# mojing1999/jmcodec

Hardware: AMD Instinct MI355X
Metric: decoded frames/sec @1080p H.264 + bit-exact YUV (higher is better)
Workload: dtype u8

## Files before the change

### jmcodec_amd/csrc/deblock_lds.hip

```cpp
#include <hip/hip_runtime.h>
#include <cstdlib>
#include <algorithm>
#include "jobs.h"
#include "kernels.h"
#include "kernel_common.h"
#include "deblock_device.h"

namespace jmamd {

__global__ __launch_bounds__(256) void k_deblock_prep(const PicParams *pics) {
    const PicParams &pp = pics[blockIdx.y];
    if (!(pp.stages & (PS_DEBLOCK_LDS | PS_CHAIN))) return;
    DbRec *out = (DbRec *)pp.dbrec;
    const int per_xcd = ((int)gridDim.x + 7) >> 3;
    const int blk = ((int)blockIdx.x & 7) * per_xcd + ((int)blockIdx.x >> 3);
    __shared__ __align__(16) uint8_t stage[8][96];
    int sub = threadIdx.x >> 5, t = threadIdx.x & 31;
    int mb = blk * 8 + sub;
    int n_mbs = pp.mb_w * pp.mb_h;
    if (mb >= n_mbs) return;
    int mbx = mb % pp.mb_w, mby = mb / pp.mb_w;
    const MbW q = load_mbw(&pp.mbs[mb]);
    const SliceRec sl = pp.slices[mbw_slice(q)];
    bool has_left = mbx > 0, has_top = mby > 0;
    MbW pl = q, pt = q;
    if (has_left) { pl = load_mbw(&pp.mbs[mb - 1]); if (sl.disable == 2 && mbw_slice(pl) != mbw_slice(q)) has_left = false; }
    if (has_top) { pt = load_mbw(&pp.mbs[mb - pp.mb_w]); if (sl.disable == 2 && mbw_slice(pt) != mbw_slice(q)) has_top = false; }
    int dir = t >> 4, e = (t >> 2) & 3, k = t & 3;
    int rq = dir == 0 ? k * 4 + e : e * 4 + k;
    int bs;
    if (sl.disable == 1) bs = 0;
    else if (e == 0) {
        bool have = dir == 0 ? has_left : has_top;
        const MbW pn = select_mbw(dir == 0, pl, pt);
        bs = have ? boundary_strength(pp, pn, dir == 0 ? k * 4 + 3 : 12 + k, q, rq, true, dir == 1) : 0;
    } else bs = boundary_strength(pp, q, dir == 0 ? rq - 1 : rq - 4, q, rq, false, dir == 1);
    if ((e & 1) && (mbw_modes(q) & MBM_T8X8)) bs = 0;
    int cls = e ? 1 : (dir ? 2 : 0);
    int qp_p = cls == 0 ? mbw_qp(pl) : (cls == 2 ? mbw_qp(pt) : mbw_qp(q)), qp_q = mbw_qp(q);
    DbRec *o = (DbRec *)stage[sub];
    {
        int qpav = (qp_p + qp_q + 1) >> 1;
        int ia = clip3(0, 51, qpav + sl.alpha_off), ib = clip3(0, 51, qpav + sl.beta_off);
        int tc0 = (bs >= 1 && bs <= 3) ? kTc0[ia][bs - 1] : 0;
        o->y_bs[t] = (uint8_t)(bs | (tc0 << 3));
        if (k == 0 && (e == 0 || (e == 1 && dir == 0))) { o->y_ab[cls][0] = kAlpha[ia]; o->y_ab[cls][1] = kBeta[ib]; }
    }
    if (!(e & 1)) {
#pragma unroll
        for (int plane = 0; plane < 2; plane++) {
            int off = plane ? pp.cr_qp_off : pp.cb_qp_off;
            int qpav = (chroma_qp(qp_p, off) + chroma_qp(qp_q, off) + 1) >> 1;
            int ia = clip3(0, 51, qpav + sl.alpha_off), ib = clip3(0, 51, qpav + sl.beta_off);
            int tc0 = (bs >= 1 && bs <= 3) ? kTc0[ia][bs - 1] : 0;
            o->c_bs[plane][dir * 8 + (e >> 1) * 4 + k] = (uint8_t)(bs | (tc0 << 3));
            if (k == 0 && (e == 0 || (e == 2 && dir == 0))) { o->c_ab[plane][cls][0] = kAlpha[ia]; o->c_ab[plane][cls][1] = kBeta[ib]; }
        }
    }
    if (t < 6) ((uint4 *)&out[mb])[t] = ((const uint4 *)stage[sub])[t];
}

template <int DEPTH>
__global__ __launch_bounds__(kBandRows * 16) void k_deblock_band(const PicParams *pics, int *ctl, int pub, int *err) {
    __shared__ __align__(16) uint8_t smem[kDeblockSmemBytes];
    const PicParams &pp = pics[blockIdx.y];
    if (!(pp.stages & PS_DEBLOCK_LDS)) return;
    deblock_band_body<DEPTH, false>(pp, blockIdx.x >> 1, blockIdx.x & 1, ctl + (size_t)blockIdx.y * kChainStride + kChainRing, pub, smem, nullptr,
        err + blockIdx.y);
}

bool deblock_lds_supported(int mb_w, int mb_h) { return mb_w > 0 && mb_h <= kBandRows * kDeblockMaxBands; }

constexpr int kDeblockDepth = 2, kDeblockPub = 2;
int deblock_depth() { return kDeblockDepth; }
int deblock_row_lag() { return kRowLag; }
int deblock_pub() { return kDeblockPub; }

void launch_deblock_prep(const PicParams *d_pics, int n, int max_mbs, hipStream_t st) {
    hipLaunchKernelGGL(k_deblock_prep, dim3(((max_mbs + 7) / 8 + 7) & ~7, n), dim3(256), 0, st, d_pics);
}
void launch_deblock_lds(const PicParams *d_pics, int n, int max_mb_h, int *ctl, int *err, bool debug_stall, hipStream_t st) {
    const int depth = deblock_depth(), pub = debug_stall ? -1 : deblock_pub();
    const int bands = (max_mb_h + kBandRows - 1) / kBandRows;
    dim3 grid(2 * bands, n), block(kBandRows * 16);
    if (depth <= 2) hipLaunchKernelGGL((k_deblock_band<2>), grid, block, 0, st, d_pics, ctl, pub, err);
    else if (depth == 3) hipLaunchKernelGGL((k_deblock_band<3>), grid, block, 0, st, d_pics, ctl, pub, err);
    else hipLaunchKernelGGL((k_deblock_band<4>), grid, block, 0, st, d_pics, ctl, pub, err);
}

}
```

### jmcodec_amd/csrc/decoder.cpp

```cpp
#include "decoder.h"
#include "numa.h"
#include <pthread.h>
#include <time.h>
#include "engine.h"
#include "host_copy.h"
#include "kernels.h"
#include <hip/hip_runtime_api.h>
#include <algorithm>
#include <cstdio>
#include <cstdlib>
#include <cstring>
#include <thread>

namespace jmamd {

#define HIP_OK(expr) ((expr) == hipSuccess)

namespace {
int thread_budget() {
    const char *e = getenv("JM_AMD_DEC_THREADS");
    int n = e ? atoi(e) : (int)std::thread::hardware_concurrency();
    if (!e) {
        if (FILE *f = fopen("/sys/fs/cgroup/cpu.max", "r")) {
            long long q = 0, per = 0; char qs[32] = {0};
            if (fscanf(f, "%31s %lld", qs, &per) == 2 && strcmp(qs, "max") != 0 && per > 0) { q = atoll(qs); int lim = (int)((q * 5 / 4 + per - 1) / per);
                if (lim < 4) lim = 4; if (n > lim) n = lim; }
            fclose(f);
        }
    }
    return std::max(1, std::min(n, 64));
}
struct Pool {
    std::mutex m; std::condition_variable cv;
    std::deque<std::pair<Decoder *, PicTask *>> q;
    std::vector<std::thread> threads;
    int n = 0, node = -1; bool bound = false;
    Pool(int node_, int n_) : n(n_), node(node_) {
        bound = (int)numa_cpus_of_node(node).size() >= std::max(2, (n * 4 / 5 + 1) / 2);
        for (int i = 0; i < n; i++) threads.emplace_back([this] { pthread_setname_np(pthread_self(),
            "jm-parse"); if (bound) numa_bind_this_thread(node); run(); });
        for (auto &t : threads) t.detach();
    }
    void run() {
        ParseScratch scratch;
        for (;;) {
            std::pair<Decoder *, PicTask *> job;
            { std::unique_lock<std::mutex> lk(m); cv.wait(lk, [&] { return !q.empty(); }); job = q.front(); q.pop_front(); }
            try { job.first->parse_task(job.second, scratch); }
            catch (const std::exception &e) { job.first->parse_exception(job.second, e.what()); }
            catch (...) { job.first->parse_exception(job.second, "unknown exception"); }
        }
    }
};
std::mutex g_pools_m;
std::vector<Pool *> g_pools;
Pool &pool_of_node(int node) {
    std::lock_guard<std::mutex> lk(g_pools_m);
    for (Pool *p : g_pools) if (p->node == node) return *p;
    int n = thread_budget();
    if (node >= 0 && !getenv("JM_AMD_DEC_DEVICE")) {
        cpu_set_t allowed; CPU_ZERO(&allowed);
        const int total = sched_getaffinity(0, sizeof allowed, &allowed) == 0 ? CPU_COUNT(&allowed) : 0;
        const int mine = (int)numa_cpus_of_node(node).size();
        if (total > 0 && mine > 0 && mine < total) n = std::max(2, (n * mine + total - 1) / total);
    }
    g_pools.push_back(new Pool(node, n));
    return *g_pools.back();
}
std::atomic<int> g_handle_counter{0};
std::atomic<int> g_handle_index{0};
}

void pool_submit(Decoder *d, PicTask *t) { Pool &p = pool_of_node(d->numa_node()); { std::lock_guard<std::mutex> lk(p.m); p.q.emplace_back(d, t); }
    p.cv.notify_one(); }
int pool_threads(int node) { return pool_of_node(node).n; }

static long long now_ns() { return std::chrono::duration_cast<std::chrono::nanoseconds>(std::chrono::steady_clock::now().time_since_epoch()).count(); }

Decoder::Decoder() { memset(info_, 0, sizeof info_); trace_on_ = getenv("JM_AMD_DEC_TRACE") != nullptr; eng_state_ = new EngineDecoderState(); }

Decoder::~Decoder() {
    { std::unique_lock<std::mutex> lk(mtx_); cv_.wait(lk, [&] { return outstanding_ == 0 && parse_pending_ == 0; }); }
    { std::lock_guard<std::mutex> lk(submit_mtx_); }
    if (copier_) { copier_->free_signal(out_sig_); out_sig_ = 0; }
    gpu_close();
    delete eng_state_;
    if (trace_on_ && !trace_.empty()) {
        char name[256]; snprintf(name, sizeof name, "%s.%p.csv", getenv("JM_AMD_DEC_TRACE"), (void *)this);
        if (FILE *f = fopen(name, "w")) {
            fprintf(f, "seq,is_i,dispatch,parsed,submit0,submit1\n");
            for (auto &r : trace_)
                fprintf(f, "%llu,%d,%lld,%lld,%lld,%lld\n", (unsigned long long)r.seq, r.is_i, r.t_dispatch, r.t_parsed, r.t_submit0, r.t_submit1);
            fclose(f);
        }
    }
}

void Decoder::fail(const std::string &msg) {
    std::lock_guard<std::mutex> lk(error_m_);
    if (!failed_) { error_ = msg; fprintf(stderr, "jm_amd_dec: %s\n", msg.c_str()); }
    failed_ = true;
}
const char *Decoder::last_error() {
    std::lock_guard<std::mutex> lk(error_m_);
    error_out_ = error_;
    return error_out_.c_str();
}

void Decoder::note_error(const std::string &msg) {
    std::lock_guard<std::mutex> lk(error_m_);
    if (!failed_) error_ = msg;
}

int Decoder::set_option(const char *key, long long v) {
    std::string k(key);
    if (k == "parse_only") parse_only_ = v != 0;
    else if (k == "digest") { want_digest_ = v != 0; if (want_digest_) sync_mode_ = true; }
    else if (k == "display_delay") display_delay_ = (int)std::max(0ll, std::min(v, (long long)n_jobs_ - 4));
    else if (k == "job_slots") { if (inited_) return -1; n_jobs_ = (int)std::max(8ll, std::min(v, (long long)kMaxJobSlots)); n_jobs_set_ = true; }
    else if (k == "fast_parse") fast_parse_ = v != 0;
    else if (k == "job_digest") { want_job_digest_ = v != 0; if (want_job_digest_) sync_mode_ = true; }
    else if (k == "sync") sync_mode_ = v != 0;
    else if (k == "device_output") device_output_ = v != 0;
    else if (k == "device") device_ = (int)v;
    else if (k == "crop_x" || k == "crop_y" || k == "crop_w" || k == "crop_h" || k == "target_width" || k == "target_height") {
        if (inited_ || v < 0 || v > 32768 || (v & 1)) return -1;
        static const char *const keys[6] = {"crop_x", "crop_y", "crop_w", "crop_h", "target_width", "target_height"};
        for (int i = 0; i < 6; i++) if (k == keys[i]) geo_[i] = (int)v;
    }
    else if (k == "rect_x" || k == "rect_y" || k == "rect_w" || k == "rect_h") {
        if (inited_ || v < 0 || v > 32768 || (v & 1)) return -1;
        rect_opt_[k[5] == 'x' ? 0 : k[5] == 'y' ? 1 : k[5] == 'w' ? 2 : 3] = (int)v;
    }
    else if (k == "fit") { if (inited_ || v < 0 || v > 2) return -1; fit_ = (int)v; }
    else if (k == "fit_sar") { if (inited_ || v < 0 || v > 1) return -1; fit_sar_ = (int)v; }
    else if (k == "fill") { if (inited_ || v < -1 || v > 0xFFFFFF) return -1; fill_ = v; }
    else if (k == "deinterlace" || k == "deinterlace_when" || k == "deinterlace_field" || k == "deinterlace_threshold") {
        const long long hi = k == "deinterlace" || k == "deinterlace_field" ? 2 : (k == "deinterlace_when" ? 1 : 255);
        if (inited_ || v < 0 || v > hi) return -1;
        (k == "deinterlace" ? deint_mode_ : k == "deinterlace_when" ? deint_when_ : k == "deinterlace_field" ? deint_field_ : deint_thr_) = (int)v;
    }
    else if (k == "deinterlace_rate") {
        if (inited_ || v < 0 || v > 1) return -1;
        deint_rate_ = (int)v;
    }
    else if (k == "verify_hash") {
        if (inited_ || v < 0 || v > 2) return -1;
        verify_hash_ = (int)v;
    }
    else if (k == "verify_md5") {
        if (inited_ || v < 0 || v > 1) return -1;
        verify_md5_ = (int)v;
    }
    else if (k == "rgb_chroma") {
        if (inited_ || v < 0 || v > 1) return -1;
        rgb_chroma_ = (int)v;
    }
    else if (k == "chroma_loc") {
        if (inited_ || v < -1 || v > 5) return -1;
        chroma_loc_opt_ = (int)v;
    }
    else if (k == "profile") { profile_ = v != 0; if (engine_) engine_->set_profile(profile_); }
    else if (k.rfind("chain_", 0) == 0 || k == "debug_stall" || k == "debug_no_bi" || k == "early_intra_ahead") {
        if (!engine_ || !engine_->set_knob(k, v)) return -1;
    }
    else if (k == "wait_idle") {
        dispatch_pending();
        { std::unique_lock<std::mutex> lk(mtx_); cv_.wait(lk, [&] { return outstanding_ == 0; }); }
    }
    else return -1;
    return 0;
}
long long Decoder::get_stat(const char *key) const {
    std::string k(key);
    if (k == "inferred_frames") return stat_inferred_frames_.load();
    if (k == "redundant_slices") return stat_redundant_slices_.load();
    if (k == "field_pictures") return stat_field_pics_.load();
    if (k == "lone_fields") return stat_lone_fields_.load();
    if (k == "frames") return num_frames_;
    if (k == "out_width") return out_w_;
    if (k == "out_height") return out_h_;
    if (k == "rect_x") return place_[0];
    if (k == "rect_y") return place_[1];
    if (k == "rect_w") return place_[2];
    if (k == "rect_h") return place_[3];
    if (k == "placed_frames") return stat_placed_;
    if (k == "sar_num") return sar_[0];
    if (k == "sar_den") return sar_[1];
    if (k == "scaled_frames") return stat_scaled_;
    if (k == "rgb_frames") return stat_rgb_;
    if (k == "deint_frames") return stat_deint_;
    if (k == "field_rate_pairs") return stat_pairs_;
    if (k == "interlaced_sequence") return codec_ == 0 && seq_active_ && !seq_.frame_mbs_only ? 1 : 0;
    if (k == "out_frame_bytes") { std::lock_guard<std::mutex> lk(const_cast<std::mutex &>(mtx_));
        return (long long)(cur_out_ ? cur_out_->fbytes : !ready_.empty() ? ready_.front()->fbytes : frame_bytes_); }
    if (k == "out_slot_bytes") { std::lock_guard<std::mutex> lk(const_cast<std::mutex &>(mtx_)); long long n = 0;
        for (const OutSlot *o : all_out_) n += (o->host ? (long long)o->bytes : 0) + (o->dev ? (long long)o->bytes : 0); return n; }
    if (k == "vui_full_range") return vui_[0];
    if (k == "vui_primaries") return vui_[1];
    if (k == "vui_transfer") return vui_[2];
    if (k == "vui_matrix") return vui_[3];
    if (k == "color_matrix") return color_matrix_;
    if (k == "color_range") return color_range_;
    if (k == "vui_chroma_loc") return vui_chroma_loc_[0];
    if (k == "vui_chroma_loc_bottom") return vui_chroma_loc_[1];
    if (k == "chroma_loc") return chroma_loc_;
    if (k == "rgb_chroma") return rgb_chroma_;
    if (k == "rgb_chroma_frames") return stat_rgb_chroma_;
    if (k == "pictures") return stat_pictures_;
    if (k == "hash_pictures") return stat_hash_pics_;
    if (k == "hash_checked") return stat_hash_checked_;
    if (k == "hash_mismatch") return stat_hash_mismatch_;
    if (k == "hash_unchecked") return stat_hash_unchecked_;
    if (k == "hash_md5") return stat_hash_md5_;
    if (k == "hash_first_bad_poc") return stat_hash_bad_poc_;
    if (k.rfind("hash_last_crc:", 0) == 0 || k.rfind("hash_last_checksum:", 0) == 0) {
        const bool crc = k[10] == 'c' && k[11] == 'r'; const int c = atoi(k.c_str() + (crc ? 14 : 19));
        return c >= 0 && c < 3 ? (long long)hash_last_[(crc ? 0 : 3) + c].load() : -1; }
    if (k.rfind("hash_last_md5:", 0) == 0) {
        const size_t c2 = k.find(':', 14); if (c2 == std::string::npos) return -1;
        const int c = atoi(k.c_str() + 14), w = atoi(k.c_str() + c2 + 1);
        return c >= 0 && c < 3 && w >= 0 && w < 4 ? (long long)hash_last_md5_[4 * c + w].load() : -1;
    }
    if (k.rfind("hash_sei_", 0) == 0) {
        const size_t colon = k.find(':'); if (colon == std::string::npos) return -1;
        const size_t i = (size_t)atoll(k.c_str() + colon + 1); if (i >= hash_seen_.size()) return -1;
        if (k.compare(0, colon, "hash_sei_md5") == 0) {
            const size_t c2 = k.find(':', colon + 1), c3 = c2 == std::string::npos ? c2 : k.find(':', c2 + 1);
            if (c3 == std::string::npos) return -1;
            const int c = atoi(k.c_str() + c2 + 1), w = atoi(k.c_str() + c3 + 1);
            if (c < 0 || c > 2 || w < 0 || w > 3) return -1;
            const uint8_t *d = hash_seen_[i].h.md5[c] + 4 * w;
            return (long long)((uint32_t)d[0] << 24 | (uint32_t)d[1] << 16 | (uint32_t)d[2] << 8 | d[3]);
        }
        if (k.compare(0, colon, "hash_sei_poc") == 0) return hash_seen_[i].poc;
        if (k.compare(0, colon, "hash_sei_type") == 0) return hash_seen_[i].h.type;
        const size_t c2 = k.find(':', colon + 1);
        if (k.compare(0, colon, "hash_sei_value") == 0 && c2 != std::string::npos) { const int c = atoi(k.c_str() + c2 + 1);
            return c >= 0 && c < 3 ? (long long)hash_seen_[i].h.v[c] : -1; }
        return -1;
    }
    if (k == "job_bytes") return stat_job_bytes_;
    if (k == "job_regrown") return stat_job_regrown_;
    if (k == "job_slot_bytes") { long long n = 0; for (auto &j : jobs_) n += (long long)j.cap; return n; }
    if (k == "errors") return stat_errors_;
    if (k == "failed") return failed_ ? 1 : 0;
    if (k == "jpeg_pictures") return stat_jpeg_pics_;
    if (k == "jpeg_sampling") return codec_ == 2 && seq_active_ ? j_sampling_ : 0;
    if (k == "jpeg_restart_intervals") return stat_jpeg_ri_;
    if (k == "copy_engines") return copier_ ? (long long)copier_->engine_mask() : 0;
    if (k == "direct_frames") return stat_direct_;
    if (k == "direct_ns") return stat_direct_ns_;
    if (k == "device_wait_errors") return stat_wait_errors_;
    if (k == "intra_mbs") return stat_intra_mbs_;
    if (k == "coef_int16") return stat_coef_;
    if (k == "syntax_digest") return codec_ == 1 ? (long long)hdigest_.h : (long long)digest_.h;
    if (k == "job_digest") return (long long)job_digest_;
    if (k == "digest_mbs") return codec_ == 1 ? (long long)hdigest_.n_cu : (long long)digest_.mbs;
    if (k == "i_pictures") return stat_i_;
    if (k == "p_pictures") return stat_p_;
    if (k == "b_pictures") return stat_b_;
    if (k == "fps_num") return codec_ == 1 ? (long long)hsps_.time_scale : (long long)seq_.time_scale;
    if (k == "fps_den") return codec_ == 1 ? (long long)hsps_.num_units_in_tick : 2ll * seq_.num_units_in_tick;
    if (k == "out_fps_num") { const bool chosen = deint_when_ == 1 || (codec_ == 0 && seq_active_ && !seq_.frame_mbs_only);
        return (field_rate() && chosen ? 2 : 1) * get_stat("fps_num"); }
    if (k == "out_fps_den") return get_stat("fps_den");
    if (k == "frames_done_unfetched") return (long long)frames_done_unfetched();
    if (k == "frames_waiting") { std::lock_guard<std::mutex> lk(const_cast<std::mutex &>(mtx_)); return (long long)ready_.size(); }
    if (k == "pictures_in_flight") { std::lock_guard<std::mutex> lk(const_cast<std::mutex &>(mtx_)); return (long long)outstanding_; }
    if (k == "coded_width") return mb_w_ * 16;
    if (k == "coded_height") return mb_h_ * 16;
    if (k == "pitch") return pitch_;
    if (k == "device") return device_;
    if (k == "threads") return pool_threads(numa_node_);
    if (k == "numa_node") return numa_node_;
    if (k == "elapsed_us") return (long long)(elapsed_ms_ * 1000.0);
    if (k == "parse_ns_i") return stat_parse_ns_i_;
    if (k == "submit_ns") return stat_submit_ns_;
    if (k == "wait_slot_ns") return stat_wait_slot_ns_;
    if (k == "parse_ns_p") return stat_parse_ns_p_;
    if (k.rfind("k_", 0) == 0 || k.rfind("eng_", 0) == 0) {
        static const char *kn[kKernelClasses] = {"inter", "intra", "deblock", "packout", "chain", "rgb_pack", "deint", "jpeg", "pichash", "md5", "rgb_pack444"};
        if (!engine_) return 0;
        EngineStats es = engine_->stats();
        for (int i = 0; i < kKernelClasses; i++) {
            if (k == std::string("k_") + kn[i] + "_ns") return (long long)es.ns[i];
            if (k == std::string("k_") + kn[i] + "_n") return es.launches[i];
            if (k == std::string("k_") + kn[i] + "_pics") return es.pics[i];
            if (k == std::string("k_") + kn[i] + "_alg_bytes") return es.alg_bytes[i];
        }
        if (k == "eng_batches") return es.batches;
        if (k == "eng_forms") return es.forms;
        if (k == "eng_form_decoders") return es.form_decoders;
        if (k == "eng_form_pending") return es.form_pending;
        if (k == "eng_batch_pics") return es.batch_pics;
        if (k == "eng_chain_batches") return es.chain_batches;
        if (k == "eng_chain_pics") return es.chain_pics;
        if (k == "eng_chain_i_batches") return es.chain_i_batches;
        if (k == "eng_wait_errors") return es.wait_errors;
        if (k == "eng_chain_recoveries") return es.chain_recoveries;
        if (k == "eng_gpu_shared") return engine_->gpu_shared() ? 1 : 0;
        if (k == "eng_launch_ns") return es.launch_ns;
        if (k == "eng_wait_gap_launches") return es.wait_gap_launches;
        if (k == "eng_wait_gap_max_us") return es.wait_gap_max_ticks / 100;
        if (k == "eng_quad_windows") return es.quad_windows;
        if (k == "eng_private_windows") return es.private_windows;
        if (k == "eng_rej_other_lane") return es.rej_other_lane;
        if (k == "eng_rej_cross_lane") return es.rej_cross_lane;
        if (k == "eng_rej_tables") return es.rej_tables;
        if (k == "eng_early_intra") return es.early_intra;
        if (k == "eng_blocked_ns") return es.blocked_ns;
        if (k == "eng_blocked_n") return es.blocked_n;
        for (int i = 0; i < 4; i++) {
            const std::string l = std::to_string(i);
            if (k == "eng_lane" + l + "_busy_ns") return (long long)es.lane_busy_ns[i];
            if (k == "eng_lane" + l + "_gap_ns") return (long long)es.lane_gap_ns[i];
            if (k == "eng_lane" + l + "_upwait_ns") return (long long)es.lane_upwait_ns[i];
            if (k == "eng_lane" + l + "_prewait_ns") return (long long)es.lane_prewait_ns[i];
            if (k == "eng_lane" + l + "_dry") return es.lane_dry[i];
            if (k == "eng_lane" + l + "_batches") return es.lane_batches[i];
            if (k == "eng_lane" + l + "_pics") return es.lane_pics[i];
        }
        if (k == "eng_complete_ns") return es.complete_ns;
        return -1;
    }
    if (k.rfind("display_field:", 0) == 0) { size_t i = (size_t)atoll(k.c_str() + 14);
        return i < display_fields_.size() ? display_fields_[i] : (i < display_pocs_.size() ? 0 : -1); }
    if (k.rfind("display_picture:", 0) == 0) { size_t i = (size_t)atoll(k.c_str() + 16);
        if (field_rate()) return i < display_pics_.size() ? (long long)display_pics_[i] : -1;
        return i < display_pocs_.size() ? (long long)i : -1; }
    if (k.rfind("display_poc:", 0) == 0) { size_t i = (size_t)atoll(k.c_str() + 12); return i < display_pocs_.size() ? display_pocs_[i] : -1; }
    return -1;
}

int Decoder::init(int codec_type, int out_fmt, const uint8_t *extra, int len) {
    codec_ = codec_type; out_fmt_ = out_fmt ? 1 : 0;
    if (codec_type != 0 && codec_type != 1 && codec_type != 2) { fail("only codec_type 0 (H.264), 1 (HEVC) and 2 (MJPEG) are implemented"); return -1; }
    if (rgb_chroma_ && !rgb_) { fail("option rgb_chroma needs RGB output: set an RGB spec (jm_amddec_set_rgb) before init"); return -1; }
    if (getenv("JM_AMD_DEC_SYNC")) sync_mode_ = true;
    if (const char *js = getenv("JM_AMD_DEC_JOB_SLOTS")) { n_jobs_ = std::max(8, std::min(atoi(js), kMaxJobSlots)); n_jobs_set_ = true; }
    if (const char *dd = getenv("JM_AMD_DEC_DISPLAY_DELAY")) display_delay_ = std::max(0, std::min(atoi(dd), n_jobs_ - 4));
    if (getenv("JM_AMD_DEC_PARSE_ONLY")) parse_only_ = true;
    out_via_copy_engine_ = !getenv("JM_AMD_DEC_OUT_DIRECT");
    if (getenv("JM_AMD_DEC_DEVICE_OUTPUT")) device_output_ = true;
    cavlc_init_tables();
    if (parse_only_) numa_node_ = numa_node_of_device(device_ < 0 ? 0 : device_, false);
    if (!parse_only_ && !gpu_open()) return -1;
    {
        int fa = 2, fb = 5;
        const char *e = getenv("JM_AMD_DEC_OUT_FETCH");
        out_route_ = 3;
        if (getenv("JM_AMD_DEC_OUT_PINNED") || !out_via_copy_engine_) out_route_ = 2;
        else if (e && !strcmp(e, "auto")) out_route_ = 0;
        else if (e && strcmp(e, "direct")) { if (sscanf(e, "%d/%d", &fa, &fb) != 2 || fb <= 0) { fa = 2; fb = 5; }
            out_route_ = (handle_index_ % fb) < fa ? 1 : 2; }
        if (out_route_ == 3 && !parse_only_) {
            copier_ = HostCopier::get(device_);
            if (copier_) out_sig_ = copier_->new_signal();
            if (!copier_ || !out_sig_) { copier_ = nullptr; out_route_ = (handle_index_ % 5) < 2 ? 1 : 2; }
        }
        out_fetch_ = out_route_ == 1 || out_route_ == 3;
        if (const char *l = getenv("JM_AMD_DEC_FETCH_LIMIT")) fetch_limit_ = atoi(l);
    }
    if (engine_) engine_->set_profile(profile_);
    inited_ = true;
    if (extra && len > 0 && codec_ == 1 && len >= 23 && extra[0] == 1) {
        avcc_len_size_ = (extra[21] & 3) + 1;
        int o = 23;
        for (int a = 0, n_arrays = extra[22]; a < n_arrays && o + 3 <= len; a++) {
            int n = (extra[o + 1] << 8) | extra[o + 2]; o += 3;
            for (int i = 0; i < n && o + 2 <= len; i++) {
                int l = (extra[o] << 8) | extra[o + 1]; o += 2;
                if (l <= 0 || o + l > len) { o = len; break; }
                handle_nal(extra + o, (size_t)l); o += l;
            }
        }
    } else if (extra && len > 0) {
        if (len >= 7 && extra[0] == 1) {
            avcc_len_size_ = (extra[4] & 3) + 1;
            int o = 5, n_sps = extra[o++] & 31;
            for (int pass = 0; pass < 2; pass++) {
                int n = pass == 0 ? n_sps : (o < len ? extra[o++] : 0);
                for (int i = 0; i < n && o + 2 <= len; i++) {
                    int l = (extra[o] << 8) | extra[o + 1]; o += 2;
                    if (l <= 0 || o + l > len) { o = len; break; }
                    handle_nal(extra + o, (size_t)l); o += l;
                }
            }
        } else { feed(extra, (size_t)len); static const uint8_t sc[4] = {0, 0, 0, 1}; feed(sc, 4); in_.clear(); scan_ = 0; have_start_ = false; }
    }
    return 0;
}

bool Decoder::gpu_open() {
    int n = 0;
    if (!HIP_OK(hipGetDeviceCount(&n)) || n <= 0) { fail("no HIP device available (the HIP backend is mandatory; there is no CPU fallback)"); return false; }
    if (device_ < 0) {
        const char *e = getenv("JM_AMD_DEC_DEVICE");
        device_ = e ? atoi(e) : (g_handle_counter++ % n);
    }
    const int named_device = device_;
    if (device_ >= n) device_ %= n;
    mem_trace("handle: before hipSetDevice");
    if (!HIP_OK(hipSetDevice(device_))) { fail("hipSetDevice failed"); return false; }
    mem_trace("handle: hipSetDevice");
    handle_index_ = g_handle_index++;
    numa_node_ = numa_node_of_device(getenv("JM_AMD_DEC_FAKE_NUMA") ? named_device : device_, true);
    engine_ = Engine::get(device_);
    if (!engine_) { fail("could not start the device engine (stream / buffer creation failed)"); return false; }
    gpu_open_ = true;
    mem_trace("handle: engine ready");
    return true;
}

void Decoder::free_job_buffers() {
    for (auto &j : jobs_) {
        if (j.big >= 0) { j.host = j.own_host; j.dev = j.own_dev; j.big = -1; }
        if (gpu_open_ && !parse_only_) { if (j.host) hipHostFree(j.host); if (j.dev) hipFree(j.dev); if (j.dbrec) hipFree(j.dbrec);
            if (j.resid) hipFree(j.resid); if (j.uploaded) hipEventDestroy(j.uploaded); }
        else free(j.host);
        j = JobSlot();
    }
    for (auto &b : big_) {
        if (gpu_open_ && !parse_only_) { if (b.host) hipHostFree(b.host); if (b.dev) hipFree(b.dev); } else free(b.host);
        b = BigJobBuf();
    }
}

void Decoder::free_surfaces() {
    if (surf_block_) hipFree(surf_block_);
    surf_block_ = nullptr;
    for (auto &p : surf_) p = nullptr;
}

void Decoder::gpu_free_sequence() {
    if (!gpu_open_) return;
    hipSetDevice(device_);
    free_surfaces();
    if (resid_) { hipFree(resid_); resid_ = nullptr; }
    for (auto &w : hevc_work_) if (w) { hipFree(w); w = nullptr; }
    if (hevc_bs_) { hipFree(hevc_bs_); hevc_bs_ = nullptr; }
    if (scale_dev_) { hipFree(scale_dev_); scale_dev_ = nullptr; }
    if (chroma_dev_) { hipFree(chroma_dev_); chroma_dev_ = nullptr; }
    free_job_buffers();
    free_out_slots(true);
}
void Decoder::free_out_slots(bool all) {
    std::lock_guard<std::mutex> lk(mtx_);
    std::vector<OutSlot *> keep;
    for (OutSlot *o : all_out_) {
        bool pending = !all && (o == cur_out_ || std::find(ready_.begin(), ready_.end(), o) != ready_.end());
        if (pending) { keep.push_back(o); continue; }
        if (o->host) hipHostFree(o->host);
        if (o->dev) hipFree(o->dev);
        delete o;
    }
    all_out_ = keep; free_out_.clear();
    if (all) { ready_.clear(); done_unfetched_ = 0; cur_out_ = nullptr; }
}
void Decoder::gpu_close() {
    if (!gpu_open_) { for (OutSlot *o : all_out_) delete o; all_out_.clear(); free_job_buffers(); return; }
    gpu_free_sequence();
    gpu_open_ = false;
}

bool upload_scale_tables(int w, int h, int tw, int th, uint8_t **dev, ScaleAxis ax[4]) {
    const int S[4] = {w, h, w / 2, h / 2}, D[4] = {tw, th, tw / 2, th / 2};
    std::vector<int32_t> first[4]; std::vector<int16_t> wt[4];
    size_t off[4][2], total = 0;
    for (int a = 0; a < 4; a++) {
        const int T = build_scale_taps(S[a], D[a], first[a], wt[a]);
        if (T < 0 || T > kScaleMaxTaps) return false;
        ax[a].taps = T; ax[a].src_len = S[a];
        off[a][0] = total; total += (first[a].size() * sizeof(int32_t) + 255) & ~(size_t)255;
        off[a][1] = total; total += (wt[a].size() * sizeof(int16_t) + 255) & ~(size_t)255;
    }
    std::vector<uint8_t> host(total, 0);
    for (int a = 0; a < 4; a++) { memcpy(host.data() + off[a][0], first[a].data(), first[a].size() * sizeof(int32_t));
        memcpy(host.data() + off[a][1], wt[a].data(), wt[a].size() * sizeof(int16_t)); }
    *dev = nullptr;
    if (!HIP_OK(hipMalloc((void **)dev, total))) { *dev = nullptr; return false; }
    if (!HIP_OK(hipMemcpy(*dev, host.data(), total, hipMemcpyHostToDevice))) { hipFree(*dev); *dev = nullptr; return false; }
    for (int a = 0; a < 4; a++) { ax[a].first = (const int32_t *)(*dev + off[a][0]); ax[a].w = (const int16_t *)(*dev + off[a][1]); }
    return true;
}

bool upload_chroma_tables(int w, int h, int tw, int th, int loc, uint8_t **dev, ScaleAxis cax[2]) {
    if (loc < 0 || loc > 5) return false;
    const int S[2] = {w / 2, h / 2}, D[2] = {tw, th}, q[2] = {chr::siting_qx(loc), chr::siting_qy(loc)};
    std::vector<int32_t> first[2]; std::vector<int16_t> wt[2];
    size_t off[2][2], total = 0;
    for (int a = 0; a < 2; a++) {
        const int T = build_chroma_taps(S[a], D[a], q[a], first[a], wt[a]);
        if (T < 0 || T > chr::kChromaMaxTaps) return false;
        cax[a].taps = T; cax[a].src_len = S[a];
        off[a][0] = total; total += (first[a].size() * sizeof(int32_t) + 255) & ~(size_t)255;
        off[a][1] = total; total += (wt[a].size() * sizeof(int16_t) + 255) & ~(size_t)255;
    }
    std::vector<uint8_t> host(total, 0);
    for (int a = 0; a < 2; a++) { memcpy(host.data() + off[a][0], first[a].data(), first[a].size() * sizeof(int32_t));
        memcpy(host.data() + off[a][1], wt[a].data(), wt[a].size() * sizeof(int16_t)); }
    *dev = nullptr;
    if (!HIP_OK(hipMalloc((void **)dev, total))) { *dev = nullptr; return false; }
    if (!HIP_OK(hipMemcpy(*dev, host.data(), total, hipMemcpyHostToDevice))) { hipFree(*dev); *dev = nullptr; return false; }
    for (int a = 0; a < 2; a++) { cax[a].first = (const int32_t *)(*dev + off[a][0]); cax[a].w = (const int16_t *)(*dev + off[a][1]); }
    return true;
}

bool color_coefs(int matrix, bool full_range, int c[5]) {
    long long kr, kb;
    switch (matrix) {
        case 1: kr = 2126; kb = 722; break;
        case 4: kr = 3000; kb = 1100; break;
        case 5: case 6: kr = 2990; kb = 1140; break;
        case 7: kr = 2120; kb = 870; break;
        case 9: kr = 2627; kb = 593; break;
        default: return false;
    }
    const long long kg = 10000 - kr - kb, syn = full_range ? 1 : 255, syd = full_range ? 1 : 219, scn = full_range ? 1 : 255, scd = full_range ? 1 : 224;
    auto rnd = [](long long n, long long d) { return (int)((2 * n + d) / (2 * d)); };
    c[0] = rnd(syn * 16384, syd);
    c[1] = rnd(scn * 2 * (10000 - kr) * 16384, scd * 10000);
    c[2] = rnd(scn * 2 * kb * (10000 - kb) * 16384, scd * 10000 * kg);
    c[3] = rnd(scn * 2 * kr * (10000 - kr) * 16384, scd * 10000 * kg);
    c[4] = rnd(scn * 2 * (10000 - kb) * 16384, scd * 10000);
    return true;
}
bool rgb_spec_valid(const RgbSpec &s, bool need_matrix) {
    const int m = s.matrix;
    return s.dtype >= RGB_U8 && s.dtype <= RGB_BF16 && (s.planar == 0 || s.planar == 1) && (s.bgr == 0 || s.bgr == 1) && s.range >= 0 && s.range <= 2 &&
           (m == 1 || m == 4 || m == 5 || m == 6 || m == 7 || m == 9 || (m == 0 && !need_matrix));
}
bool fill_rgb_color(RgbJob &j, const RgbSpec &s, int matrix, bool full_range) {
    int c[5];
    if (!color_coefs(matrix, full_range, c)) return false;
    j.cy = c[0]; j.crv = c[1]; j.cgu = c[2]; j.cgv = c[3]; j.cbu = c[4]; j.yo = full_range ? 0 : 16;
    j.dtype = s.dtype; j.planar = s.planar; j.bgr = s.bgr;
    for (int k = 0; k < 3; k++) { j.k[k] = s.scale[k] * (1.0f / 16384.0f); j.b[k] = s.bias[k]; }
    return true;
}

int Decoder::set_rgb(const RgbSpec *spec) {
    if (inited_) return -1;
    if (!spec) { rgb_ = false; return 0; }
    if (!rgb_spec_valid(*spec, false)) return -1;
    rgb_spec_ = *spec; rgb_ = true;
    return 0;
}

void Decoder::resolve_color(const int vui[4], int disp_h) {
    for (int i = 0; i < 4; i++) vui_[i] = vui[i];
    int m = rgb_ ? rgb_spec_.matrix : 0, c[5];
    if (m == 0) m = vui[3] >= 0 && color_coefs(vui[3], false, c) ? vui[3] : (disp_h > 576 ? 1 : 6);
    const int r = rgb_ && rgb_spec_.range ? rgb_spec_.range : (vui[0] == 1 ? 2 : 1);
    color_matrix_ = m; color_range_ = r;
}

bool Decoder::resolve_chroma_loc(int vui_top, int vui_bottom, int fallback) {
    vui_chroma_loc_[0] = vui_top; vui_chroma_loc_[1] = vui_bottom;
    const int loc = chroma_loc_opt_ >= 0 ? chroma_loc_opt_ : (vui_top >= 0 && vui_top <= 5 ? vui_top : fallback);
    const bool changed = loc != chroma_loc_;
    chroma_loc_ = loc;
    return changed && rgb_chroma_ && rgb_;
}

bool fit_rect(int cw, int ch, int sar_num, int sar_den, int tw, int th, int fit, int rect[4]) {
    if (!rect || cw <= 0 || ch <= 0 || tw < 2 || th < 2 || ((tw | th) & 1) || sar_num < 0 || sar_den < 0 || (fit != 1 && fit != 2)) return false;
    if (cw > 32768 || ch > 32768 || tw > 32768 || th > 32768 || sar_num > 65535 || sar_den > 65535) return false;
    const long long sn = sar_num && sar_den ? sar_num : 1, sd = sar_num && sar_den ? sar_den : 1;
    const long long Wp = cw * sn, Hp = ch * sd, TW = tw, TH = th;
    auto clampll = [](long long v, long long lo, long long hi) { return v < lo ? lo : (v > hi ? hi : v); };
    long long rw, rh;
    if (Wp * TH >= Hp * TW) { rw = TW; rh = clampll(2 * ((TW * Hp + Wp) / (2 * Wp)), 2, TH); }
    else { rh = TH; rw = clampll(2 * ((TH * Wp + Hp) / (2 * Hp)), 2, TW); }
    rect[0] = fit == 1 ? (int)(2 * ((TW - rw) / 4)) : 0; rect[1] = fit == 1 ? (int)(2 * ((TH - rh) / 4)) : 0;
    rect[2] = (int)rw; rect[3] = (int)rh;
    return true;
}

bool Decoder::resolve_geometry() {
    const int W = disp_w_, H = disp_h_;
    out_w_ = W; out_h_ = H; crop_[0] = crop_[1] = 0; crop_[2] = W; crop_[3] = H; scaled_ = false;
    place_[0] = place_[1] = 0; place_[2] = W; place_[3] = H; placed_ = false; rgb_identity_ = true;
    const bool rect_set = (rect_opt_[0] | rect_opt_[1] | rect_opt_[2] | rect_opt_[3]) != 0;
    if (!(geo_[0] | geo_[1] | geo_[2] | geo_[3] | geo_[4] | geo_[5]) && !rect_set && !fit_) return true;
    const int cx = geo_[0], cy = geo_[1], cw = geo_[2] ? geo_[2] : W - cx, ch = geo_[3] ? geo_[3] : H - cy;
    const int tw = geo_[4] ? geo_[4] : cw, th = geo_[5] ? geo_[5] : ch;
    char msg[256];
    if (cw <= 0 || ch <= 0 || cx + cw > W || cy + ch > H) {
        snprintf(msg, sizeof msg, "output geometry: the crop rectangle %dx%d at (%d, %d) does not lie inside the display area %dx%d", cw, ch, cx, cy, W, H);
        fail(msg); return false;
    }
    if ((cw | ch) & 1) {
        snprintf(msg, sizeof msg, "output geometry: the crop size %dx%d (display area %dx%d) is odd", cw, ch, W, H);
        fail(msg); return false;
    }
    int rc[4] = {0, 0, tw, th};
    if (fit_) {
        if (!geo_[4] || !geo_[5]) { fail("output geometry: fit needs both target_width and target_height"); return false; }
        if (rect_set) { fail("output geometry: fit and rect_x / rect_y / rect_w / rect_h exclude each other"); return false; }
        if (!fit_rect(cw, ch, fit_sar_ ? sar_[0] : 0, fit_sar_ ? sar_[1] : 0, tw, th, fit_, rc)) { fail("output geometry: fit: no rectangle for this target"); return false; }
    } else if (rect_set) {
        rc[0] = rect_opt_[0]; rc[1] = rect_opt_[1]; rc[2] = rect_opt_[2] ? rect_opt_[2] : tw - rc[0]; rc[3] = rect_opt_[3] ? rect_opt_[3] : th - rc[1];
        if (rc[2] <= 0 || rc[3] <= 0 || rc[0] + rc[2] > tw || rc[1] + rc[3] > th) {
            snprintf(msg, sizeof msg, "output geometry: the placement rectangle %dx%d at (%d, %d) does not lie inside the target %dx%d", rc[2], rc[3], rc[0], rc[1], tw, th);
            fail(msg); return false;
        }
    }
    if (cw > 8 * rc[2] || ch > 8 * rc[3] || rc[2] > 4 * cw || rc[3] > 4 * ch) {
        snprintf(msg, sizeof msg, "output geometry: the scaling ratio %dx%d -> %dx%d is out of range (per axis at most 8:1 down and 1:4 up)", cw, ch, rc[2], rc[3]);
        fail(msg); return false;
    }
    crop_[0] = cx; crop_[1] = cy; crop_[2] = cw; crop_[3] = ch; out_w_ = tw; out_h_ = th;
// ... 771 lines not shown
}

int Decoder::acquire_job_slot(bool big) {
    auto w0 = std::chrono::steady_clock::now();
    std::unique_lock<std::mutex> lk(mtx_);
    const bool lend = big && codec_ == 0 && big_[0].host != nullptr;
    int got = -1, bg = -1;
    cv_.wait(lk, [&] {
        got = -1;
        for (int i = 0; i < n_jobs_; i++) if (!jobs_[i].busy && (got < 0 || (big ? jobs_[i].cap > jobs_[got].cap : jobs_[i].cap < jobs_[got].cap))) got = i;
        return got >= 0;
    });
    if (lend && jobs_[got].cap < job_cap_max_) for (int i = 0; i < kBigJobBufs && bg < 0; i++) if (!big_[i].busy) bg = i;
    if (bg >= 0) {
        JobSlot &j = jobs_[got];
        j.own_host = j.host; j.own_dev = j.dev; j.own_cap = j.cap;
        j.host = big_[bg].host; j.dev = big_[bg].dev; j.cap = job_cap_max_; j.big = bg; big_[bg].busy = true;
    }
    jobs_[got].busy = true;
    stat_wait_slot_ns_ += std::chrono::duration_cast<std::chrono::nanoseconds>(std::chrono::steady_clock::now() - w0).count();
    return got;
}

void Decoder::push_task(std::unique_ptr<PicTask> t) {
    PicTask *raw = t.get();
    if (sync_mode_) { std::unique_lock<std::mutex> lk(mtx_); cv_.wait(lk, [&] { return outstanding_ == 0; }); }
    raw->t_dispatch = now_ns();
    {
        std::lock_guard<std::mutex> lk(mtx_);
        raw->seq = next_seq_++;
        outstanding_++;
        if (raw->has_picture) parse_pending_++;
        inflight_.push_back(std::move(t));
    }
    if (raw->has_picture) pool_submit(this, raw);
    else { raw->state.store(1, std::memory_order_release); submit_ready(); }
}

void Decoder::parse_task(PicTask *t, ParseScratch &scratch) {
    if (t->hevc) { hevc_parse_task(t); return; }
    if (t->jpeg) { jpeg_parse_task(t); return; }
    auto pt0 = std::chrono::steady_clock::now();
    JobSlot &js = jobs_[t->job_slot];
    const int n_mbs = t->sps.mb_w * t->sps.mb_h;
    scratch.resize(t->sps.mb_w, t->sps.mb_h);
    scratch.begin_picture();
    static thread_local std::vector<int16_t> mv_ext_buf;
    const bool big_rec = t->sps.profile_idc != 66;
    mv_ext_buf.resize((size_t)n_mbs * (big_rec ? kBiRecInt16 : 32));
    const size_t fixed = (size_t)n_mbs * sizeof(MbRec) + 256 * sizeof(SliceRec);
    MbRec *mbs = nullptr; SliceRec *srec = nullptr; int16_t *coef = nullptr;
    MbRec blank; memset(&blank, 0, sizeof blank); blank.kind = MB_INTER;
    { int8_t c = -1; for (auto &s : t->slices) if (s.sh.type != SL_I && s.refs.slot[0][0] >= 0) { c = s.refs.slot[0][0]; break; }
      blank.ref[0] = blank.ref[1] = blank.ref[2] = blank.ref[3] = c; }
    JobWriter w;
    SyntaxDigest dg = digest_;
    for (int attempt = 0;; attempt++) {
        scratch.begin_picture();
        mbs = (MbRec *)js.host; srec = (SliceRec *)(js.host + (size_t)n_mbs * sizeof(MbRec)); coef = (int16_t *)(srec + 256);
        w = JobWriter();
        w.mbs = mbs; w.mv_ext = mv_ext_buf.data(); w.mv_ext_cap = (uint32_t)n_mbs * (big_rec ? kBiRecInt16 / 2 : 16);
        w.coef = coef;
        {
            long long room = (long long)js.cap - (long long)fixed - 64;
            if (room <= 0) { t->error = "job buffer too small for this picture"; stat_errors_++; fail(t->error); room = 0; }
            w.coef_cap = (uint32_t)(room / 2);
        }
        dg = digest_;
        t->n_intra = 0; t->n_i8x8 = 0; t->any_deblock = false; t->any_wp = false; t->error.clear();
        const char *first_error = nullptr; bool overflow = false;
        for (size_t si = 0; si < t->slices.size(); si++) {
            SliceTask &s = t->slices[si];
            srec[si].alpha_off = (int8_t)s.sh.alpha_off; srec[si].beta_off = (int8_t)s.sh.beta_off; srec[si].disable = (uint8_t)s.sh.disable_deblock;
            srec[si].pad = 0;
            if (s.sh.disable_deblock != 1) t->any_deblock = true;
            BitReader br(s.rbsp.data(), s.rbsp_len);
            br.set_end_from_trailing();
            br.skip_bytes(s.sh.data_bit_offset >> 3); br.skip((int)(s.sh.data_bit_offset & 7));
            if (s.sh.first_mb >= n_mbs) { t->error = "first_mb_in_slice out of range"; continue; }
            if (s.col) s.col->wait();
            if (s.has_wp) t->any_wp = true;
            SliceParseResult r = parse_slice_data(t->sps, t->pps, s.sh, br, (int)si, s.refs, scratch, w, want_digest_ ? &dg : nullptr, fast_parse_ &&
                !t->field);
            t->n_intra += r.n_intra; t->n_i8x8 += r.n_i8x8;
            if (r.error) { t->error = r.error; if (!first_error) first_error = r.error; overflow |= strcmp(r.error, "coefficient buffer overflow") == 0; }
        }
        if (overflow && js.cap < job_cap_max_ && attempt < 6 && !failed_) {
            const bool i_pic = !t->slices.empty() && t->slices[0].sh.type == SL_I;
            const size_t want = std::min(job_cap_max_, std::max(js.cap * 2, i_pic ? i_job_peak_.load() * 5 / 4 : (size_t)0));
            if (ensure_job_cap(js, want)) { stat_job_regrown_++; continue; }
        }
        if (!t->error.empty()) { stat_errors_++; note_error(std::string("slice data: ") + t->error); }
        break;
    }
    for (int i = 0; i < n_mbs; i++) if (scratch.slice_of[i] < 0) mbs[i] = blank;
    if (want_digest_) digest_ = dg;
    if (const char *dm = getenv("JM_AMD_DEC_DUMP_MB")) {
        int dp = 0, dx = 0, dy = 0;
        if (sscanf(dm, "%d:%d:%d", &dp, &dx, &dy) == 3 && (dp < 0 || dp == (int)stat_pictures_.load())) {
            for (int oy = -1; oy <= 0; oy++) for (int ox = -1; ox <= 1; ox++) {
                const int x = dx + ox, y = dy + oy;
                if (x < 0 || y < 0 || x >= t->sps.mb_w || y >= t->sps.mb_h || (oy == 0 && ox == 1)) continue;
                const MbRec &m = mbs[y * t->sps.mb_w + x];
                fprintf(stderr, "MB(%d,%d) kind %d flags 0x%02x modes 0x%02x qp %d slice %d cbp_blk 0x%04x i4 %02x%02x%02x%02x%02x%02x%02x%02x "
                        "n_intra %d n_i8x8 %d slice_type %d\n", x, y, m.kind, m.flags, m.modes, m.qp, m.slice, m.cbp_blk,
                        m.u.i4[0], m.u.i4[1], m.u.i4[2], m.u.i4[3], m.u.i4[4], m.u.i4[5], m.u.i4[6], m.u.i4[7], t->n_intra, t->n_i8x8,
                            t->slices.empty() ? -1 : (int)t->slices[0].sh.type);
            }
        }
    }
    t->n_slices = (int)t->slices.size();
    if (t->mf) {
        MotionField &f = *t->mf;
        size_t n = (size_t)n_mbs;
        f.mv[0].assign(scratch.mv.begin(), scratch.mv.begin() + n * 32); f.mv[1].assign(scratch.mv1.begin(), scratch.mv1.begin() + n * 32);
        f.ref[0].assign(scratch.refidx.begin(), scratch.refidx.begin() + n * 4); f.ref[1].assign(scratch.refidx1.begin(), scratch.refidx1.begin() + n * 4);
        f.uid[0].assign(scratch.uid0.begin(), scratch.uid0.begin() + n * 4); f.uid[1].assign(scratch.uid1.begin(), scratch.uid1.begin() + n * 4);
        f.intra.resize(n);
        for (size_t i = 0; i < n; i++) f.intra[i] = scratch.slice_of[i] < 0 || (scratch.info[i] & 1);
        f.publish();
    }
    if (w.coef_count & 1) w.coef[w.coef_count++] = 0;
    {
        const size_t need = fixed + (size_t)w.coef_count * 2 + (size_t)w.mv_ext_count * 4 + (t->any_wp ? t->slices.size() * sizeof(SliceWp) : 0) + 64;
        if (need > js.cap) {
            if (!ensure_job_cap(js, std::min(need + need / 4, std::max(job_cap_max_, need)),
                fixed + (size_t)w.coef_count * 2)) fail("job buffer allocation failed");
            else { mbs = (MbRec *)js.host; srec = (SliceRec *)(js.host + (size_t)n_mbs * sizeof(MbRec)); coef = (int16_t *)(srec + 256); w.mbs = mbs;
                w.coef = coef; stat_job_regrown_++; }
        }
    }
    if (failed_) { w.mv_ext_count = 0; }
    memcpy(w.coef + w.coef_count, mv_ext_buf.data(), (size_t)w.mv_ext_count * 4);
    t->coef_count = w.coef_count; t->mv_ext_count = w.mv_ext_count; t->max_mvy = w.max_mvy; t->max_mvx = w.max_mvx;
    t->upload_bytes = fixed + (size_t)w.coef_count * 2 + (size_t)w.mv_ext_count * 4;
    if (want_job_digest_) {
        uint64_t h = job_digest_;
        auto eat = [&](const void *p, size_t n) { const uint8_t *b = (const uint8_t *)p; for (size_t i = 0; i < n; i++) { h ^= b[i]; h *= 1099511628211ull; } };
        eat(mbs, (size_t)n_mbs * sizeof(MbRec)); eat(srec, t->slices.size() * sizeof(SliceRec));
        eat(w.coef, (size_t)w.coef_count * 2 + (size_t)w.mv_ext_count * 4);
        const int mm = w.max_mvy, mmx = w.max_mvx; eat(&mm, sizeof mm); eat(&mmx, sizeof mmx);
        job_digest_ = h;
    }
    if (t->any_wp && t->upload_bytes + t->slices.size() * sizeof(SliceWp) > js.cap) { t->error = "job buffer overflow (weight tables)"; stat_errors_++;
        t->any_wp = false; }
    if (t->any_wp) {
        t->wp_offset = t->upload_bytes;
        for (auto &s : t->slices) { if (!s.has_wp) memset(&s.wp, 0, sizeof s.wp); memcpy(js.host + t->upload_bytes, &s.wp, sizeof(SliceWp));
            t->upload_bytes += sizeof(SliceWp); }
    }
    stat_pictures_++; stat_job_bytes_ += (long long)t->upload_bytes; stat_intra_mbs_ += t->n_intra; stat_coef_ += w.coef_count;
    for (auto &s : t->slices) { std::vector<uint8_t>().swap(s.rbsp); }
    if (!parse_only_ && !failed_) {
        t->upload_seq = engine_->upload(js.dev, js.host, t->upload_bytes, js.uploaded);
    }
    {
        long long ns = std::chrono::duration_cast<std::chrono::nanoseconds>(std::chrono::steady_clock::now() - pt0).count();
        bool is_i = !t->slices.empty() && t->slices[0].sh.type == SL_I;
        (is_i ? stat_parse_ns_i_ : stat_parse_ns_p_) += ns;
        if (is_i) { size_t pk = i_job_peak_.load(); while (t->upload_bytes + 4096 > pk && !i_job_peak_.compare_exchange_weak(pk, t->upload_bytes + 4096)) {} }
    }
    t->t_parsed = now_ns();
    t->state.store(1, std::memory_order_release);
    submit_ready();
    { std::lock_guard<std::mutex> lk(mtx_); parse_pending_--; cv_.notify_all(); }
}

void Decoder::parse_exception(PicTask *t, const char *what) {
    fail(std::string("exception while parsing a picture: ") + what);
    stat_errors_++;
    t->error = what;
    t->state.store(1, std::memory_order_release);
    submit_ready();
    { std::lock_guard<std::mutex> lk(mtx_); parse_pending_--; cv_.notify_all(); }
}

void Decoder::submit_ready() {
    std::lock_guard<std::mutex> sl(submit_mtx_);
    for (;;) {
        std::unique_ptr<PicTask> t;
        {
            std::lock_guard<std::mutex> lk(mtx_);
            if (inflight_.empty() || inflight_.front()->state.load(std::memory_order_acquire) != 1) break;
            t = std::move(inflight_.front());
            inflight_.pop_front();
        }
        long long ts0 = now_ns();
        submit_task(t.get());
        if (trace_on_ && t->has_picture) trace_.push_back(TraceRec{t->seq, t->t_dispatch, t->t_parsed, ts0, now_ns(), (!t->slices.empty() &&
            t->slices[0].sh.type == SL_I) ? 1 : 0});
    }
}

int Decoder::display_entry(int slot) {
    const DpbPic &d = dpb_[slot];
    int field = 0, both = 0;
    if (deint_mode_) {
        if (d.deint) field = d.lone ? d.lone : (deint_field_ ? deint_field_ : (codec_ == 0 && d.fpoc[1] < d.fpoc[0] ? 2 : 1));
        display_fields_.push_back((uint8_t)field);
        both = deint_rate_ && field && !d.lone;
        if (both) display_fields_.push_back((uint8_t)(3 - field));
        if (deint_rate_) display_pics_.insert(display_pics_.end(), both ? 2 : 1, display_count_);
    }
    display_count_++;
    return slot | d.lone << 8 | d.color << 16 | field << 24 | both << 26;
}

void Decoder::enqueue_output(int entry, OutSide &out) {
    const int slot = entry & 255, color = (entry >> 16) & 255, field = (entry >> 24) & 3, both = (entry >> 26) & 1;
    int lone = (entry >> 8) & 255;
    OutSlot *o, *o2 = nullptr;
    { std::lock_guard<std::mutex> lk(mtx_); o = alloc_out_slot(); ready_.push_back(o); num_frames_++;
      if (both) { o2 = alloc_out_slot(); ready_.push_back(o2); num_frames_++; } }
    if (both) stat_pairs_++;
    if (placed_ && !failed_) stat_placed_ += both ? 2 : 1;
    if (parse_only_ || failed_) { std::lock_guard<std::mutex> lk(mtx_); o->ready = true; done_unfetched_++; if (field) stat_deint_++;
        if (both) { o2->ready = true; done_unfetched_++; stat_deint_++; } return; }
    auto dst_of = [](OutSlot *s) { return s->dev ? s->dev : s->host; };
    const uint8_t *src = surf_[slot]; int src_chroma = chroma_off_;
    if (field) {
        const int t = deint_thr_ ? deint_thr_ : 10;
        DeintReq r{DeintJob{surf_[slot], dst_of(o), pitch_, chroma_off_, disp_w_, disp_h_, disp_w_, disp_w_ * disp_h_, out_fmt_, lone ? 1 : deint_mode_,
                            field - 1, 4 * t * t, both ? dst_of(o2) : nullptr}, 0, 0, 0};
        if (rgb_ || scaled_) {
            r.feeds = rgb_ ? 2 : 1; r.index = (int)(rgb_ ? out.rgb.size() : out.scale.size()); r.index2 = both ? r.index + 1 : 0;
            r.job.dst = r.job.dst2 = nullptr; r.job.dst_pitch = pitch_; r.job.dst_chroma_offset = src_chroma = pitch_ * disp_h_; r.job.out_fmt = 0;
            src = nullptr; lone = 0;
        }
        out.deint.push_back(r); stat_deint_ += both ? 2 : 1;
    }
    for (OutSlot *s : {o, o2}) {
        if (!s) continue;
        if (rgb_) {
            RgbJob rj = {};
            rj.s = ScaleJob{src, dst_of(s), pitch_, src_chroma, crop_[0], crop_[1], out_w_, out_h_, 0, lone, {}};
            for (int a = 0; a < 4; a++) rj.s.ax[a] = scale_ax_[a];
            rj.identity = rgb_identity_ ? 1 : 0;
            if (rgb_chroma_) { rj.identity = 0; rj.chroma = 1; rj.cax[0] = chroma_ax_[0]; rj.cax[1] = chroma_ax_[1]; stat_rgb_chroma_++; }
            if (placed_) { rj.s.rx = place_[0]; rj.s.ry = place_[1]; rj.s.rw = place_[2]; rj.s.rh = place_[3]; rj.fill = fill_ < 0 ? 0 : (int)fill_; }
            fill_rgb_color(rj, rgb_spec_, color & 15, (color >> 4) == 2);
            out.rgb.push_back(rj); stat_rgb_++;
            if (scaled_ && !rgb_identity_) stat_scaled_++;
        } else if (scaled_) {
            ScaleJob sj{src, dst_of(s), pitch_, src_chroma, crop_[0], crop_[1], out_w_, out_h_, out_fmt_, lone, {}};
            for (int a = 0; a < 4; a++) sj.ax[a] = scale_ax_[a];
            if (placed_) { sj.rx = place_[0]; sj.ry = place_[1]; sj.rw = place_[2]; sj.rh = place_[3]; sj.fill = fill_ < 0 ? 0x108080 : (int)fill_; }
            out.scale.push_back(sj); stat_scaled_++;
        } else if (!field) out.plain.push_back(PackJob{surf_[slot], dst_of(s), pitch_, chroma_off_, disp_w_, disp_h_, out_fmt_, lone});
        out.slots.push_back(s);
        s->has_data = true;
        s->fetch = s->dev && (!s->host || (out_route_ == 0 && engine_ && engine_->fetchers() < fetch_limit_));
    }
}

void Decoder::submit_task(PicTask *t) {
    auto st0 = std::chrono::steady_clock::now();
    EnginePic ep;
    ep.dec = this; ep.has_picture = t->has_picture && !parse_only_ && !failed_; ep.job_slot = t->job_slot;
    ep.mb_w = mb_w_; ep.mb_h = mb_h_; ep.disp_w = disp_w_; ep.disp_h = disp_h_; ep.wait_prev_pack = t->wait_prev_pack;
    for (int s : t->out_before) { enqueue_output(s, ep.out[kBefore]); ep.out_mask |= 1u << (s & 255); }
    memset(&ep.pp, 0, sizeof ep.pp);
    if (ep.has_picture && t->hevc) hevc_fill_engine_pic(t, ep);
    else if (t->hevc && (t->hevc->hash.type > 0 || (t->hevc->hash.type == 0 && verify_md5_)) && !parse_only_) stat_hash_unchecked_++;
    else if (ep.has_picture && t->jpeg) jpeg_fill_engine_pic(t, ep);
    else if (ep.has_picture) {
        JobSlot &js = jobs_[t->job_slot];
        const int n_mbs = t->sps.mb_w * t->sps.mb_h;
        PicParams &pp = ep.pp;
        ep.uploaded = js.uploaded; ep.upload_seq = t->upload_seq;
        pp.mb_w = t->sps.mb_w; pp.mb_h = t->sps.mb_h; pp.mb_w_magic = (uint32_t)(((1ull << 32) + (uint32_t)pp.mb_w - 1) / (uint32_t)pp.mb_w);
        pp.surf_stride = (uint32_t)(surf_[1] - surf_[0]);
        pp.pitch = t->field ? 2 * pitch_ : pitch_; pp.chroma_offset = chroma_off_; pp.field = t->field;
        ep.mb_h = t->sps.mb_h;
        pp.cb_qp_off = t->pps.chroma_qp_off; pp.cr_qp_off = t->pps.second_chroma_qp_off;
        pp.n_slices = t->n_slices; pp.cur = t->cur_slot;
        for (int i = 0; i < kMaxSurfaces; i++) pp.surf[i] = surf_[i];
        pp.surf_base = surf_block_;
        pp.mbs = (const MbRec *)js.dev;
        pp.slices = (const SliceRec *)(js.dev + (size_t)n_mbs * sizeof(MbRec));
        pp.coef = (const int16_t *)(pp.slices + 256);
        pp.mv_ext = pp.coef + t->coef_count;
        pp.resid = (int16_t *)js.resid; pp.dbrec = js.dbrec;
        pp.wp = t->any_wp ? (const SliceWp *)(js.dev + t->wp_offset) : nullptr;
        {
            static const uint8_t zz4[16] = {0, 1, 4, 8, 5, 2, 3, 6, 9, 12, 13, 10, 7, 11, 14, 15};
            static const uint8_t zz8[64] = {0, 1, 8, 16, 9, 2, 3, 10, 17, 24, 32, 25, 18, 11, 4, 5, 12, 19, 26, 33, 40, 48, 41, 34, 27, 20, 13, 6, 7, 14, 21,
                28,
                                            35, 42, 49, 56, 57, 50, 43, 36, 29, 22, 15, 23, 30, 37, 44, 51, 58, 59, 52, 45, 38, 31, 39, 46, 53, 60, 61, 54, 47,
                                                55, 62, 63};
            bool flat = true;
            for (int i = 0; i < 6; i++) for (int k = 0; k < 16; k++) { pp.wscale4[i][zz4[k]] = t->pps.scaling4[i][k]; flat &= t->pps.scaling4[i][k] == 16; }
            for (int i = 0; i < 2; i++) for (int k = 0; k < 64; k++) { pp.wscale8[i][zz8[k]] = t->pps.scaling8[i][k]; flat &= t->pps.scaling8[i][k] == 16; }
            pp.flat_scaling = flat ? 1 : 0;
        }
        bool lds_intra = use_lds_intra_ && t->n_intra * 16 >= n_mbs && (t->n_i8x8 == 0 || lds_intra8_);
        pp.want_intra_resid = lds_intra ? 1 : 0;
        pp.stages = PS_RECON;
        if (t->n_intra > 0) pp.stages |= lds_intra ? PS_INTRA_LDS : PS_INTRA_V1;
        if (t->any_deblock) pp.stages |= use_lds_deblock_ ? PS_DEBLOCK_LDS : PS_DEBLOCK_V1;
        ep.chain_ok = chain_ok_ && pp.stages == (PS_RECON | PS_DEBLOCK_LDS) && t->n_intra == 0 && !t->field;
        ep.chain_intra = chain_ok_ && chain_intra_on_ && t->n_intra > 0 && use_lds_intra_ && (t->n_i8x8 == 0 || lds_intra8_) && (pp.stages & PS_DEBLOCK_LDS) &&
                         !t->field;
        ep.classic_stages = pp.stages;
        for (auto &sl : t->slices) ep.bipred |= sl.refs.bipred_rec;
        ep.reach_rows = ((t->max_mvy >> 2) + 15) / 16;
        ep.reach_cols = ((t->max_mvx >> 2) + 15) / 16;
        for (auto &sl : t->slices) for (int l = 0; l < 2; l++) for (int i = 0; i < 32; i++) if (sl.refs.slot[l][i] >= 0) ep.ref_mask |=
            1u << (sl.refs.slot[l][i] & 31);
        long long S = (long long)surf_bytes_;
        bool is_i = !t->slices.empty() && t->slices[0].sh.type == SL_I;
        ep.alg_bytes[0] = (is_i ? 0 : 2 * S) + (long long)t->upload_bytes;
        ep.alg_bytes[1] = is_i ? S : (long long)t->n_intra * 384;
        ep.alg_bytes[2] = 2 * S;
    }
    ep.alg_bytes[3] = (scaled_ || rgb_ ? (long long)crop_[2] * crop_[3] * 3 / 2 : (long long)surf_bytes_) + (long long)frame_bytes_;
    ep.alg_bytes[4] = 2ll * disp_w_ * disp_h_ * 3 / 2;
    for (int s : t->out_after) { enqueue_output(s, ep.out[kAfter]); ep.out_mask |= 1u << (s & 255); }
    stat_submit_ns_ += std::chrono::duration_cast<std::chrono::nanoseconds>(std::chrono::steady_clock::now() - st0).count();
    if (parse_only_ || failed_ || !engine_) { on_engine_done(ep); return; }
    engine_->submit(std::move(ep));
}

void Decoder::on_device_wait_error(int code) {
    stat_errors_++; stat_wait_errors_++;
    if (code & 64) note_error("device: a kernel met a motion record it was compiled without (code " + std::to_string(code) + "): the picture is damaged");
    else note_error("device: a wait between workgroups timed out (code " + std::to_string(code) + "): the picture may be damaged");
}

void Decoder::on_picture_hash(const EnginePic &p, const uint32_t *words, int bad) {
    if (!words) { stat_hash_unchecked_++; return; }
    for (int k = 0; k < 6; k++) hash_last_[k] = words[k];
    stat_hash_checked_++;
    if (bad < 0) return;
    if (stat_hash_mismatch_++ == 0) stat_hash_bad_poc_ = p.hash_poc;
    static const char *const comp[3] = {"Y", "Cb", "Cr"};
    char msg[160];
    snprintf(msg, sizeof msg, "picture hash mismatch: POC %d, component %s, %s expected 0x%x got 0x%x", p.hash_poc, comp[bad],
             p.hash_type == 1 ? "crc" : "checksum", p.hash_want[bad], words[(p.hash_type == 1 ? 0 : 3) + bad]);
    if (verify_hash_ == 2) fail(msg); else note_error(msg);
}

void Decoder::on_picture_md5(const EnginePic &p, const uint8_t *digests, int bad) {
    for (int k = 0; k < 12; k++) { const uint8_t *d = digests + 4 * k; hash_last_md5_[k] = (uint32_t)d[0] << 24 | (uint32_t)d[1] << 16 | (uint32_t)d[2] << 8 | d[3]; }
    stat_hash_checked_++;
    if (bad < 0) return;
    if (stat_hash_mismatch_++ == 0) stat_hash_bad_poc_ = p.hash_poc;
    static const char *const comp[3] = {"Y", "Cb", "Cr"};
    char want[33], got[33], msg[192];
    for (int k = 0; k < 16; k++) { snprintf(want + 2 * k, 3, "%02x", p.md5_want[bad][k]); snprintf(got + 2 * k, 3, "%02x", digests[16 * bad + k]); }
    snprintf(msg, sizeof msg, "picture hash mismatch: POC %d, component %s, md5 expected %s got %s", p.hash_poc, comp[bad], want, got);
    if (verify_hash_ == 2) fail(msg); else note_error(msg);
}

void Decoder::on_engine_done(const EnginePic &p, bool failed) {
    if (failed) { stat_errors_++; fail("device error: the batch holding this handle's picture did not complete"); }
    {
        std::lock_guard<std::mutex> lk(mtx_);
        if (p.job_slot >= 0) {
            JobSlot &j = jobs_[p.job_slot];
            if (j.big >= 0) { big_[j.big].busy = false; j.host = j.own_host; j.dev = j.own_dev; j.cap = j.own_cap; j.big = -1; }
            j.busy = false;
        }
        for (auto &side : p.out) for (OutSlot *o : side.slots) { o->ready = true; if (failed) o->has_data = false; }
        done_unfetched_ += (int)(p.out[kBefore].slots.size() + p.out[kAfter].slots.size());
        outstanding_--;
        cv_.notify_all();
    }
}

int Decoder::pop_output(bool block, int wait_us) {
    std::unique_lock<std::mutex> lk(mtx_);
    if (cur_out_) { free_out_.push_back(cur_out_); cur_out_ = nullptr; }
    const auto deadline = std::chrono::steady_clock::now() + std::chrono::microseconds(wait_us > 0 ? wait_us : 0);
    auto nap = [&] { return wait_us > 0 && cv_.wait_until(lk, deadline) != std::cv_status::timeout; };
    for (;;) {
        if (!ready_.empty()) {
            OutSlot *o = ready_.front();
            if (!block && outstanding_ < display_delay_ && (int)ready_.size() <= 6) return 0;
            if (!o->ready) { if (!block) { if (nap()) continue; return 0; } cv_.wait(lk); continue; }
            ready_.pop_front(); done_unfetched_--;
            cur_out_ = o;
            return 1;
        }
        if (outstanding_ == 0) return 0;
        if (!block) { if (nap()) continue; return 0; }
        cv_.wait(lk);
    }
}

int Decoder::poll(int *got_frame, int wait_us) {
    *got_frame = 0;
    if (!inited_ || failed_) return -1;
    *got_frame = pop_output(false, wait_us);
    return 0;
}

int Decoder::push(const uint8_t *buf, int len) {
    if (!inited_ || failed_ || !buf || len <= 0) return -1;
    if (!eos_sent_ && !eof_flag_) feed(buf, (size_t)len);
    return failed_ ? -1 : 0;
}

int Decoder::push_eos() {
    if (!inited_ || failed_) return -1;
    if (!eos_sent_) { flush_stream(); eos_sent_ = true; }
    return failed_ ? -1 : 0;
}

int Decoder::decode(const uint8_t *buf, int len, int *got_frame) {
    *got_frame = 0;
    if (!inited_ || failed_) return -1;
    if (!eos_sent_) {
        if (buf && len > 0 && !eof_flag_) feed(buf, (size_t)len);
        else { eos_sent_ = true; flush_stream(); }
    }
    if (failed_) return -1;
    bool block = eos_sent_ || sync_mode_;
    if (sync_mode_ && !eos_sent_) { std::unique_lock<std::mutex> lk(mtx_); cv_.wait(lk, [&] { return outstanding_ == 0; }); }
    int got = pop_output(block);
    *got_frame = got;
    if (!got && (eos_sent_ || eof_flag_)) {
        bool drained;
        { std::lock_guard<std::mutex> lk(mtx_); drained = outstanding_ == 0 && ready_.empty(); }
        if (drained && eos_sent_ && !is_exit_) {
            elapsed_ms_ = timer_started_ ? std::chrono::duration<double, std::milli>(std::chrono::steady_clock::now() - t0_).count() : 0.0;
            is_exit_ = true;
            char fmt[96];
            if (rgb_) { static const char *const dt[4] = {"u8", "f32", "f16", "bf16"};
                char loc[40] = "";
                if (rgb_chroma_) snprintf(loc, sizeof loc, ", chroma interpolated (loc %d)", chroma_loc_);
                snprintf(fmt, sizeof fmt, "%s %s %s%s", rgb_spec_.bgr ? "BGR" : "RGB", rgb_spec_.planar ? "planar" : "interleaved", dt[rgb_spec_.dtype & 3], loc); }
            else snprintf(fmt, sizeof fmt, "%s", out_fmt_ == 0 ? "NV12" : "YV12");
            char deint[96] = "";
            if (deint_mode_) snprintf(deint, sizeof deint, "Deinterlace:\t%s, %s%s, %lld frames\n", deint_mode_ == 1 ? "bob" : "comb-adaptive",
                deint_when_ ? "always" : "auto", deint_rate_ ? ", field rate" : "", (long long)stat_deint_);
            char place[64] = "";
            if (placed_) snprintf(place, sizeof place, "Placement:\t%d,%d %dx%d\n", place_[0], place_[1], place_[2], place_[3]);
            snprintf(info_, sizeof info_,
                     "==========================================\n"
                     "Codec:\t\t%s\n"
                     "Display:\t%d x %d\n"
                     "Pixel Format:\t%s\n"
                     "%s%s"
                     "Frame Count:\t%d\n"
                     "Elapsed Time:\t%d ms\n"
                     "Decode FPS:\t%f fps\n"
                     "==========================================\n",
                     codec_ == 0 ? "H.264" : (codec_ == 1 ? "H.265" : "MJPEG"), out_w_, out_h_, fmt, deint, place, (int)num_frames_,
                     (int)elapsed_ms_, elapsed_ms_ > 0 ? (double)num_frames_ * 1000.0 / elapsed_ms_ : 0.0);
        }
    }
    return 0;
}

int Decoder::output(uint8_t *out, int *out_len) {
    if (!cur_out_ || (!cur_out_->has_data && !parse_only_)) return -1;
    int need = (int)cur_out_->fbytes;
    if (*out_len < need) return -2;
    *out_len = 0;
    if (cur_out_->has_data && cur_out_->host && !cur_out_->fetch) memcpy(out, cur_out_->host, (size_t)need);
    else if (cur_out_->has_data) {
        hipSetDevice(device_);
        const auto c0 = std::chrono::steady_clock::now();
        void *dst = out_route_ == 3 && copier_ ? copier_->lock(out, (size_t)need) : nullptr;
        const HostCopier::Result cr = dst ? copier_->copy(dst, cur_out_->dev, (size_t)need, out_sig_) : HostCopier::kNotSubmitted;
        if (cr == HostCopier::kStuck) { fail("device: a frame copy into the caller's buffer never completed (device hung?)"); return -1; }
        if (dst) copier_->unlock(out);
        const bool went = cr == HostCopier::kDone;
        if (went) { stat_direct_++; stat_direct_ns_ += std::chrono::duration_cast<std::chrono::nanoseconds>(std::chrono::steady_clock::now() - c0).count(); }
        else {
            if (engine_) engine_->fetch_begin();
            const hipError_t ce = hipMemcpy(out, cur_out_->dev, (size_t)need, hipMemcpyDeviceToHost);
            if (engine_) engine_->fetch_end();
            if (ce != hipSuccess) return -1;
        }
    }
    else memset(out, 0, (size_t)need);
    *out_len = need;
    return need;
}

int Decoder::output_device(void **dev, int *len) {
    if (!cur_out_ || !cur_out_->has_data || !cur_out_->dev) return -1;
    *dev = cur_out_->dev; *len = (int)cur_out_->fbytes;
    return *len;
}
int Decoder::output_argb_device(void *dev_dst, int pitch) {
    if (rgb_) return -1;
    if (!cur_out_ || !cur_out_->has_data || !cur_out_->dev || pitch < cur_out_->w * 4) return -1;
    hipSetDevice(device_);
    launch_frame_to_argb(cur_out_->dev, cur_out_->w, cur_out_->h, out_fmt_, (uint8_t *)dev_dst, pitch, nullptr);
    return hipStreamSynchronize(nullptr) == hipSuccess ? 0 : -1;
}

int Decoder::stream_info(int *w, int *h) const {
    if (cur_out_) { *w = cur_out_->w; *h = cur_out_->h; return 0; }
    *w = out_w_; *h = out_h_;
    return 0;
}

int Decoder::output_nv12_pitch_device(void *dev_dst, int pitch) {
    if (rgb_) return -1;
    if (!cur_out_ || !cur_out_->has_data || !cur_out_->dev || pitch < cur_out_->w) return -1;
    hipSetDevice(device_);
    launch_frame_to_nv12_pitch(cur_out_->dev, cur_out_->w, cur_out_->h, out_fmt_, (uint8_t *)dev_dst, pitch, nullptr);
    return hipStreamSynchronize(nullptr) == hipSuccess ? 0 : -1;
}

}
```

### jmcodec_amd/csrc/engine.cpp

```cpp
#include "engine.h"
#include <sys/prctl.h>
#include "chain_order.h"
#include "decoder.h"
#include "kernels.h"
#include "hevc_kernels.h"
#include "numa.h"
#include <hip/hip_runtime_api.h>
#include <pthread.h>
#include <algorithm>
#include <chrono>
#include <cstdio>
#include <cstring>
#include <cstdlib>

namespace jmamd {

static long g_lane_trace = getenv("JM_AMD_DEC_LANE_TRACE") ? atol(getenv("JM_AMD_DEC_LANE_TRACE")) : 0;
static double trace_ms() { static const auto t0 = std::chrono::steady_clock::now();
    return std::chrono::duration<double, std::milli>(std::chrono::steady_clock::now() - t0).count(); }
#define LANE_TRACE(...) do { if (g_lane_trace > 0) { g_lane_trace--; fprintf(stderr, "lane-trace %9.3f " , trace_ms()); fprintf(stderr, __VA_ARGS__); } } while (0)

static std::mutex g_engines_m;
static Engine *g_engines[64] = {nullptr};

Engine *Engine::get(int device) {
    std::lock_guard<std::mutex> lk(g_engines_m);
    if (device < 0 || device >= 64) return nullptr;
    if (!g_engines[device]) {
        Engine *e = new Engine(device);
        if (!e->ok_) return nullptr;
        g_engines[device] = e;
    }
    return g_engines[device];
}

void mem_trace(const char *tag) {
    static const bool on = getenv("JM_AMD_DEC_MEMTRACE") != nullptr;
    if (!on) return;
    long pages = 0, res = 0;
    if (FILE *f = fopen("/proc/self/statm", "r")) { if (fscanf(f, "%ld %ld", &pages, &res) != 2) res = 0; fclose(f); }
    fprintf(stderr, "jm_amd_dec: memtrace %-44s %8.1f MB resident\n", tag, res * 4096.0 / 1e6);
}

Engine::Engine(int device) : device_(device) {
    (void)trace_ms();
    mem_trace("engine: start");
    if (const char *e = getenv("JM_AMD_DEC_CHAIN_DEPTH")) { chain_depth_ = std::max(1, std::min(atoi(e), 16)); chain_depth_few_ = chain_depth_.load(); }
    if (const char *e = getenv("JM_AMD_DEC_CHAIN_STREAMS")) chain_max_streams_ = std::max(0, atoi(e));
    if (const char *e = getenv("JM_AMD_DEC_CHAIN_LAG")) chain_lag_steps_ = std::max(kMinChainLag, std::min(atoi(e), 1024));
    if (const char *e = getenv("JM_AMD_DEC_CHAIN_LINGER")) chain_linger_streams_ = std::max(0, atoi(e));
    if (const char *e = getenv("JM_AMD_DEC_CROSS_LANE")) cross_lane_ = atoi(e) != 0;
    if (const char *e = getenv("JM_AMD_DEC_FILL_LINGER_US")) fill_linger_ns_ = std::max(0, atoi(e)) * 1000ll;
    if (const char *e = getenv("JM_AMD_DEC_EARLY_INTRA")) early_intra_ = atoi(e) != 0;
    if (hipSetDevice(device_) != hipSuccess) return;
    if (const char *e = getenv("JM_AMD_DEC_COPY_STREAMS")) n_copy_ = std::max(1, std::min(atoi(e), 4));
    int prio_lo = 0, prio_hi = 0, copy_prio = 0;
    hipDeviceGetStreamPriorityRange(&prio_lo, &prio_hi);
    { const char *e = getenv("JM_AMD_DEC_COPY_PRIORITY"); const int want = e ? atoi(e) : 1;
      copy_prio = want > 0 ? prio_hi : (want < 0 ? prio_lo : 0); }
    for (int k = 0; k < n_copy_; k++) if (hipStreamCreateWithPriority(&copy_streams_[k], hipStreamNonBlocking, copy_prio) != hipSuccess) {
        (void)hipGetLastError();
        if (hipStreamCreateWithFlags(&copy_streams_[k], hipStreamNonBlocking) != hipSuccess) return; }
    mem_trace("engine: copy stream");
    for (auto &ln : lanes_) {
        hipStream_t s, p, q;
        if (hipStreamCreateWithFlags(&s, hipStreamNonBlocking) != hipSuccess || hipStreamCreateWithFlags(&p, hipStreamNonBlocking) != hipSuccess ||
            hipStreamCreateWithFlags(&q, hipStreamNonBlocking) != hipSuccess) return;
        ln.stream = s; ln.pack_stream = p; ln.pre_stream = q;
        mem_trace("engine: lane streams");
        for (auto &b : ln.ring) {
            if (hipHostMalloc((void **)&b.h_pics, sizeof(PicParams) * kMaxBatch, hipHostMallocDefault) != hipSuccess) return;
            if (hipMalloc((void **)&b.d_pics, sizeof(PicParams) * kMaxBatch) != hipSuccess) return;
            if (hipHostMalloc((void **)&b.h_hpics, sizeof(HevcPicParams) * kMaxBatch, hipHostMallocDefault) != hipSuccess) return;
            if (hipMalloc((void **)&b.d_hpics, sizeof(HevcPicParams) * kMaxBatch) != hipSuccess) return;
            if (hipMalloc((void **)&b.d_progress, sizeof(int) * kMaxBatch * kHevcProgressStride) != hipSuccess) return;
            if (hipMalloc((void **)&b.d_ctl, sizeof(int) * ((size_t)kMaxBatch * chain_ctl_ints() + chain_tail_ints())) != hipSuccess) return;
            if (hipHostMalloc((void **)&b.h_err, sizeof(int) * (kMaxBatch + 4), hipHostMallocMapped) != hipSuccess) return;
            if (hipHostGetDevicePointer((void **)&b.d_err, b.h_err, 0) != hipSuccess) return;
            memset(b.h_err, 0, sizeof(int) * (kMaxBatch + 4));
            if (hipHostMalloc((void **)&b.h_groups, sizeof(uint32_t) * kMaxChainGroups, hipHostMallocDefault) != hipSuccess) return;
            if (hipMalloc((void **)&b.d_groups, sizeof(uint32_t) * kMaxChainGroups) != hipSuccess) return;
            bool tables_ok = true;
            b.out.each([&](auto &t) { const size_t bytes = sizeof(*t.host) * 2 * kOutSideCap;
                tables_ok = tables_ok && hipHostMalloc((void **)&t.host, bytes, hipHostMallocDefault) == hipSuccess &&
                            hipMalloc((void **)&t.dev, bytes) == hipSuccess; });
            if (!tables_ok) return;
            if (hipEventCreateWithFlags(&b.done, hipEventDisableTiming) != hipSuccess) return;
            if (hipEventCreateWithFlags(&b.kdone, hipEventDisableTiming) != hipSuccess) return;
            if (hipEventCreateWithFlags(&b.packed, hipEventDisableTiming) != hipSuccess) return;
            if (hipEventCreateWithFlags(&b.pre_done, hipEventDisableTiming) != hipSuccess) return;
            for (auto &e : b.pev) if (hipEventCreate(&e) != hipSuccess) return;
        }
    }
    mem_trace("engine: lane buffers");
    { const int r = chain_resident_workgroups(false), ri = chain_resident_workgroups(true);
      if (r > 0) chain_bands_max_ = std::min(kMaxChainBands, r / 2);
      if (ri > 0) chain_bands_max_intra_ = std::min(kMaxChainBandsIntra, ri / 2);
      if (getenv("JM_AMD_DEC_VERBOSE")) fprintf(stderr,
          "jm_amd_dec: device %d holds %d / %d chain workgroups (plain / with the intra role): band budget %d / %d\n", device_, r, ri, chain_bands_max_,
          chain_bands_max_intra_); }
    mem_trace("engine: occupancy queries");
    ok_ = true;
    numa_node_ = numa_node_of_device(device_, true);
    kfd_gpu_id_ = getenv("JM_AMD_DEC_IGNORE_SHARED_GPU") ? 0 : kfd_gpu_id_of_device(device_);
    th_ = std::thread([this] { pthread_setname_np(pthread_self(), "jm-engine"); numa_bind_this_thread(numa_node_); run(); });
    th_.detach();
}

unsigned long long Engine::upload(uint8_t *dev, const uint8_t *host, size_t n, ihipEvent_t *ev, bool spread) {
    std::lock_guard<std::mutex> lk(um_);
    hipSetDevice(device_);
    unsigned long long seq = ++upload_seq_;
    if (!spread) while (seq % (unsigned)n_copy_) seq = ++upload_seq_;
    hipStream_t cs = copy_streams_[seq % (unsigned)n_copy_];
    hipMemcpyAsync(dev, host, n, hipMemcpyHostToDevice, cs);
    hipEventRecord(ev, cs);
    return seq;
}

void Engine::submit(EnginePic &&p) {
    {
        std::lock_guard<std::mutex> lk(m_);
        if (p.codec == 0) {
            const long long now = std::chrono::duration_cast<std::chrono::nanoseconds>(std::chrono::steady_clock::now().time_since_epoch()).count();
            auto it = std::find_if(recent_.begin(), recent_.end(), [&](const Recent &r) { return r.dec == p.dec; });
            if (it == recent_.end()) { recent_.push_back(Recent{p.dec, now, 0}); it = recent_.end() - 1; }
            it->t = now;
            if (p.has_picture) it->mbs = p.mb_w * p.mb_h;
        }
        p.seq = p.dec->engine_state().next_seq++;
        if (p.dec->engine_state().n_pending++ == 0) decoders_pending_++;
        pending_.push_back(std::move(p));
        pending_gen_++;
    }
    cv_.notify_one();
}

bool Engine::set_knob(const std::string &key, long long v) {
    if (key.rfind("chain_", 0) == 0) { chain_block_until_ns_ = 0; shared_checked_ns_ = 0; }
    if (key == "chain_depth") { if (v <= 0) { chain_depth_ = 8; chain_depth_few_ = 16; }
        else { chain_depth_ = (int)std::min(v, 16ll); chain_depth_few_ = chain_depth_.load(); } }
    else if (key == "chain_lag") chain_lag_steps_ = (int)std::max((long long)kMinChainLag, std::min(v, 1024ll));
    else if (key == "chain_streams") chain_max_streams_ = (int)std::max(0ll, v);
    else if (key == "debug_stall") debug_stall_ = (int)v;
    else if (key == "debug_no_bi") debug_no_bi_ = (int)v;
    else if (key == "early_intra_ahead") early_intra_ahead_ = (int)std::max(1ll, std::min(v, 64ll));
    else return false;
    return true;
}

EngineStats Engine::stats() { std::lock_guard<std::mutex> lk(sm_); return st_; }

bool Engine::others_done(Decoder *d, int lane_idx, unsigned long long seq) {
    for (int li = 0; li < kLanes; li++) {
        if (li == lane_idx) continue;
        Lane &o = lanes_[li];
        for (int k = 0; k < o.inflight; k++) {
            Batch &ob = o.ring[(o.tail + k) % kBatchRing];
            bool mine = false;
            for (auto &p : ob.pics) if (p.dec == d && p.seq < seq) { mine = true; break; }
            if (mine && hipEventQuery(ob.packed) != hipSuccess) { (void)hipGetLastError(); return false; }
        }
    }
    return true;
}

void Engine::inflight_masks(Decoder *d, uint32_t &touched) {
    touched = 0;
    for (auto &o : lanes_) for (int k = 0; k < o.inflight; k++) for (auto &p : o.ring[(o.tail + k) % kBatchRing].pics) if (p.dec == d) {
        touched |= p.ref_mask | p.out_mask;
        if (p.has_picture) touched |= 1u << (p.codec == 0 ? p.pp.cur : p.hp.cur);
    }
}

bool Engine::form(Lane &ln, int lane_idx, Batch &b) {
    b.pics.clear(); b.any_chain = false; b.chain_with_intra = false; b.max_depth = 1;
    bool chaining = false;
    int depth_now = chain_depth_;
    {
        const long long now = std::chrono::duration_cast<std::chrono::nanoseconds>(std::chrono::steady_clock::now().time_since_epoch()).count();
        recent_.erase(std::remove_if(recent_.begin(), recent_.end(), [&](const Recent &r) { return now - r.t > 50ll * 1000 * 1000; }), recent_.end());
        const int n_active = (int)recent_.size();
        double load = 0;
        for (const Recent &r : recent_) load += std::max(1.0, r.mbs / 8160.0);
        chaining = chain_depth_ > 1 && n_active > 0 && load <= (double)chain_max_streams_ && now >= chain_block_until_ns_ &&
            !gpu_shared_.load(std::memory_order_relaxed);
        depth_now = n_active <= chain_linger_streams_ ? std::max(chain_depth_.load(), chain_depth_few_.load()) : chain_depth_.load();
        if (lane_idx == kOrdinaryLane && chaining && n_active <= chain_linger_streams_ && ln.inflight > 0) {
            int n = 0;
            for (const EnginePic &p : pending_) if (p.codec == 0 && p.has_picture && p.lane(true) == lane_idx) n++;
            if (n < depth_now * n_active) return false;
        }
    }
    if (lane_idx == kOrdinaryLane && !chaining && fill_linger_ns_ > 0 && (int)recent_.size() > decoders_pending_) {
        const long long now = std::chrono::duration_cast<std::chrono::nanoseconds>(std::chrono::steady_clock::now().time_since_epoch()).count();
        if (!ln.wait_since_ns) ln.wait_since_ns = now;
        if (now - ln.wait_since_ns < fill_linger_ns_) {
            bool urgent = false; size_t n_seen = 0; const size_t n_dec = (size_t)decoders_pending_;
            scan_tag_form_++;
            for (auto it = pending_.begin(); it != pending_.end() && n_seen < n_dec && !urgent; ++it) {
                EngineDecoderState &es = it->dec->engine_state();
                if (es.form_tag == scan_tag_form_) continue;
                es.form_tag = scan_tag_form_; n_seen++;
                if (it->lane(false) != lane_idx || es.inflight > es.lane_inflight[lane_idx]) continue;
                urgent = it->dec->frames_done_unfetched() < 1;
            }
            if (!urgent) { lingered_ = true; return false; }
        }
    }
    if (lane_idx == kOrdinaryLane) ln.wait_since_ns = 0;
    if (lane_idx == kIntraLane && !chaining && !deep_queues_ && fill_linger_ns_ > 0) {
        const long long now = std::chrono::duration_cast<std::chrono::nanoseconds>(std::chrono::steady_clock::now().time_since_epoch()).count();
        if (!ln.wait_since_ns || now - ln.wait_since_ns < fill_linger_ns_) {
            bool urgent = false; int n_elig = 0; size_t n_seen = 0; const size_t n_dec = (size_t)decoders_pending_;
            scan_tag_form_++;
            for (auto it = pending_.begin(); it != pending_.end() && n_seen < n_dec && !urgent && n_elig < 4; ++it) {
                EngineDecoderState &es = it->dec->engine_state();
                if (es.form_tag == scan_tag_form_) continue;
                es.form_tag = scan_tag_form_; n_seen++;
                if (it->codec != 0 || it->lane(false) != lane_idx) continue;
                if (es.inflight > es.lane_inflight[lane_idx] && !(cross_lane_ && others_done(it->dec, lane_idx, it->seq))) continue;
                n_elig++;
                urgent = it->dec->frames_done_unfetched() < 1;
            }
            if (n_elig == 0) return false;
            if (!ln.wait_since_ns) ln.wait_since_ns = now;
            if (n_elig < 4 && !urgent && now - ln.wait_since_ns < fill_linger_ns_) { lingered_ = true; return false; }
        }
        ln.wait_since_ns = 0;
    }
    std::vector<Decoder *> seen, members;
    const bool relaxed = cross_lane_ && !chaining;
    const long long now_ns = std::chrono::duration_cast<std::chrono::nanoseconds>(std::chrono::steady_clock::now().time_since_epoch()).count();
    size_t n_pre = 0, n_post = 0;
    auto account = [&](EnginePic &p, EngineDecoderState &es) {
        if (p.has_picture) es.batch_written |= 1u << (p.codec == 0 ? p.pp.cur : p.hp.cur);
        es.batch_read |= p.ref_mask | p.out_mask;
        n_pre += p.out[kBefore].frames(); n_post += p.out[kAfter].frames();
    };
    const size_t n_dec_pending = (size_t)decoders_pending_;
    auto took = [&](EngineDecoderState &es) { if (--es.n_pending == 0) decoders_pending_--; };
    for (auto it = pending_.begin(); it != pending_.end() && (int)b.pics.size() < kMaxBatch && seen.size() < n_dec_pending;) {
        Decoder *d = it->dec;
        if (std::find(seen.begin(), seen.end(), d) != seen.end()) { ++it; continue; }
        seen.push_back(d);
        EngineDecoderState &es = d->engine_state();
        int why = 0;
        if (it->lane(chaining) != lane_idx) why = 1;
        else if (es.inflight > es.lane_inflight[lane_idx] && !(relaxed && others_done(d, lane_idx, it->seq))) why = 2;
        else if (n_pre + it->out[kBefore].frames() > (size_t)kOutSideCap || n_post + it->out[kAfter].frames() > (size_t)kOutSideCap) why = 3;
        if (why) {
            if (lane_idx == kOrdinaryLane && it->codec == 0) { std::lock_guard<std::mutex> lk(sm_);
                (why == 1 ? st_.rej_other_lane : why == 2 ? st_.rej_cross_lane : st_.rej_tables)++;
                if (!es.blocked_since) { es.blocked_since = now_ns;
                    if (g_lane_trace > 0) {
                        LANE_TRACE("left-out dec %p seq %llu why %d inflight %d (lane0 %d lane1 %d)\n", (void *)d, it->seq, why, es.inflight, es.lane_inflight[0],
                            es.lane_inflight[1]);
                        for (int li = 0; li < kLanes; li++) for (int k = 0; k < lanes_[li].inflight; k++) { Batch &ob = lanes_[li].ring[(lanes_[li].tail + k) % kBatchRing];
                            for (auto &p : ob.pics) if (p.dec == d) LANE_TRACE("    in flight: lane %d batch %llu seq %llu kdone %d packed %d done %d\n", li, ob.serial, p.seq,
                                (int)hipEventQuery(ob.kdone), (int)hipEventQuery(ob.packed), (int)hipEventQuery(ob.done)); }
                        (void)hipGetLastError();
                    } } }
            ++it; continue;
        }
        if (lane_idx == kOrdinaryLane && es.blocked_since) { std::lock_guard<std::mutex> lk(sm_); st_.blocked_ns += now_ns - es.blocked_since; st_.blocked_n++;
            LANE_TRACE("rejoined dec %p seq %llu after %.3f ms\n", (void *)d, it->seq, (now_ns - es.blocked_since) * 1e-6);
            es.blocked_since = 0; }
        es.inflight++; es.lane_inflight[lane_idx]++;
        es.in_batch = 1; es.batch_written = es.batch_read = 0; es.batch_stop = false;
        account(*it, es);
        members.push_back(d);
        took(es);
        b.pics.push_back(std::move(*it));
        it = pending_.erase(it);
    }
    if (lane_idx == kIntraLane && early_intra_ && deep_queues_ && !chaining && early_scanned_gen_ != pending_gen_ && now_ns - early_scan_ns_ > 250 * 1000) {
        early_scan_ns_ = now_ns;
        const unsigned long long tag = ++early_scan_tag_;
        std::vector<std::deque<EnginePic>::iterator> cand;
        for (auto it = pending_.begin(); it != pending_.end(); ++it) {
            Decoder *d = it->dec;
            EngineDecoderState &es = d->engine_state();
            if (es.scan_tag != tag) { es.scan_tag = tag; es.scan_touched = 0; es.scan_ahead = 0;
                es.scan_closed = std::find(members.begin(), members.end(), d) != members.end(); }
            const uint32_t own = it->has_picture ? 1u << (it->codec == 0 ? it->pp.cur : it->hp.cur) : 0u;
            if (!es.scan_closed && it->codec == 0 && it->has_picture && it->lane(false) == kIntraLane && it->ref_mask == 0 && it->before_empty() &&
                !it->wait_prev_pack && !(it->out_mask & ~own)) {
                es.scan_closed = true;
                uint32_t infl; inflight_masks(d, infl);
                const bool landed = !it->uploaded || hipEventQuery(it->uploaded) == hipSuccess;
                if (!landed) (void)hipGetLastError();
                if (landed && es.scan_ahead >= early_intra_ahead_.load() && !(own & (es.scan_touched | infl))) cand.push_back(it);
            }
            es.scan_touched |= it->ref_mask | it->out_mask | own;
            es.scan_ahead++;
        }
        if (!cand.empty()) {
            std::vector<size_t> pos;
            for (auto &c : cand) pos.push_back((size_t)(c - pending_.begin()));
            for (size_t k = pos.size(); k-- > 0 && (int)b.pics.size() < kMaxBatch;) {
                auto it = pending_.begin() + (std::ptrdiff_t)pos[k];
                if (n_post + it->out[kAfter].frames() > (size_t)kOutSideCap) continue;
                EngineDecoderState &es = it->dec->engine_state();
                es.inflight++; es.lane_inflight[lane_idx]++;
                LANE_TRACE("early dec %p seq %llu\n", (void *)it->dec, it->seq);
                n_post += it->out[kAfter].frames();
                took(es);
                b.pics.push_back(std::move(*it));
                pending_.erase(it);
                { std::lock_guard<std::mutex> lk(sm_); st_.early_intra++; }
            }
        }
        early_scanned_gen_ = pending_gen_;
    }
    if (b.pics.empty()) return false;
    pending_gen_++;
    if (lane_idx == kOrdinaryLane) {
        { std::lock_guard<std::mutex> lk(sm_); st_.forms++; st_.form_decoders += (long long)seen.size(); st_.form_pending += (long long)(pending_.size() + b.pics.size()); }
        const size_t depth = (pending_.size() + b.pics.size()) / std::max<size_t>(1, seen.size());
        if (depth >= 16) deep_queues_ = true; else if (depth <= 8) deep_queues_ = false;
    }
    auto chain_cost = [&](const EnginePic &p, int &bands, int &groups) { bands = (p.chain_intra ? 4 : 2) * ((p.mb_h + 15) / 16);
        groups = p.mb_h * ((p.mb_w + 7) / 8) + 2 * ((p.mb_h + 15) / 16); };
    int tot_bands = 0, tot_groups = 0; bool any_intra = false;
    for (auto &p : b.pics) if (p.has_picture && (p.chain_ok || p.chain_intra)) { int nb, ng; chain_cost(p, nb, ng); tot_bands += nb; tot_groups += ng;
        any_intra |= p.chain_intra; }
    auto band_limit = [&](bool intra) { return intra ? chain_bands_max_intra_ : chain_bands_max_; };
    if (lane_idx == kOrdinaryLane && chaining && (int)members.size() <= chain_max_streams_ && tot_bands <= band_limit(any_intra) &&
        tot_groups <= kMaxChainGroups) {
        const int depth_cap = std::min(depth_now, std::max(1, kMaxBatch / (int)members.size()));
        for (int depth = 1; depth < depth_cap; depth++) {
            bool added = false;
            for (Decoder *d : members) {
                EngineDecoderState &es = d->engine_state();
                if (es.batch_stop || (int)b.pics.size() >= kMaxBatch) continue;
                auto it = std::find_if(pending_.begin(), pending_.end(), [&](const EnginePic &p) { return p.dec == d; });
                const bool ok = it != pending_.end() && it->lane(true) == lane_idx && it->has_picture && (it->chain_ok || it->chain_intra) &&
                                it->before_empty() && !it->wait_prev_pack &&
                                !((1u << it->pp.cur) & (es.batch_written | es.batch_read)) && n_post + it->out[kAfter].frames() <= (size_t)kOutSideCap;
                int nb = 0, ng = 0;
                if (ok) chain_cost(*it, nb, ng);
                if (!ok || tot_bands + nb > band_limit(any_intra || it->chain_intra) || tot_groups + ng > kMaxChainGroups) { es.batch_stop = true; continue; }
                tot_bands += nb; tot_groups += ng; any_intra |= it->chain_intra;
                es.inflight++; es.lane_inflight[lane_idx]++; es.in_batch++;
                account(*it, es);
                took(es);
                b.pics.push_back(std::move(*it));
                pending_.erase(it);
                b.any_chain = true; added = true;
            }
            if (!added) break;
            b.max_depth = depth + 1;
        }
    }
    if (lane_idx == kHevcLane || lane_idx == kHevcIntraLane) {
        for (Decoder *d : members) {
            EngineDecoderState &es = d->engine_state();
            while (es.in_batch < kHevcWorkSets && (int)b.pics.size() < kMaxBatch) {
                auto it = std::find_if(pending_.begin(), pending_.end(), [&](const EnginePic &p) { return p.dec == d; });
                if (it == pending_.end() || !it->has_picture || it->codec == 0 || it->lane(false) != lane_idx || !it->before_empty() ||
                    it->wait_prev_pack) break;
                if ((it->ref_mask & es.batch_written) || ((1u << it->hp.cur) & (es.batch_written | es.batch_read)) ||
                    n_post + it->out[kAfter].frames() > (size_t)kOutSideCap) break;
                es.inflight++; es.lane_inflight[lane_idx]++; es.in_batch++;
                es.batch_written |= 1u << it->hp.cur;
                account(*it, es);
                took(es);
                b.pics.push_back(std::move(*it));
                pending_.erase(it);
            }
        }
    }
    return true;
}

void Engine::launch(Lane &ln, Batch &b) {
    const int n = (int)b.pics.size(), li = (int)(&ln - lanes_);
    b.serial = ++ln.launched; b.last_ev = -1;
    b.launched_dry = false;
    if (profile_) {
        const Batch &pb = ln.ring[(ln.head + kBatchRing - 1) % kBatchRing];
        if (pb.serial + 1 == b.serial && pb.kdone) { const bool ended = hipEventQuery(pb.kdone) == hipSuccess; (void)hipGetLastError();
            b.launched_dry = ended;
            if (ended) { std::lock_guard<std::mutex> lk(sm_); st_.lane_dry[li]++; } }
    }
    LANE_TRACE("launch lane %d batch %llu pics %d\n", li, b.serial, n);
    int max_mbs = 0, max_mb_h = 0, max_mb_w = 0, stages = 0;
    bool wait_pack = false, any_hevc = false, any_jpeg = false; int max_jpeg_items = 0;
    for (auto &p : b.pics) any_jpeg |= p.codec == 2 && p.has_picture;
    if (any_jpeg && !b.h_jpics) {
        if (hipHostMalloc((void **)&b.h_jpics, sizeof(JpegPicParams) * kMaxBatch, hipHostMallocDefault) != hipSuccess ||
            hipMalloc((void **)&b.d_jpics, sizeof(JpegPicParams) * kMaxBatch) != hipSuccess) {
            (void)hipGetLastError();
            if (b.h_jpics) hipHostFree(b.h_jpics);
            b.h_jpics = nullptr; b.d_jpics = nullptr; any_jpeg = false;
            for (auto &p : b.pics) if (p.codec == 2 && p.has_picture) { p.has_picture = false; p.dec->on_engine_error("hipMalloc(MJPEG parameter table) failed"); }
        }
    }
    if (any_jpeg && profile_ && !b.jev[0]) for (auto &e : b.jev) if (hipEventCreate(&e) != hipSuccess) { (void)hipGetLastError(); e = nullptr; }
    b.any_hash = false;
    for (auto &p : b.pics) b.any_hash |= p.codec == 1 && p.has_picture && p.hp.hash_mode != 0;
    if (b.any_hash && !b.d_hash) {
        const size_t bytes = sizeof(uint32_t) * kMaxBatch * kHashStride;
        if (hipMalloc((void **)&b.d_hash, bytes) != hipSuccess || hipHostMalloc((void **)&b.h_hash, bytes, hipHostMallocDefault) != hipSuccess) {
            (void)hipGetLastError();
            if (b.d_hash) hipFree(b.d_hash);
            b.d_hash = nullptr; b.h_hash = nullptr; b.any_hash = false;
            for (auto &p : b.pics) p.hp.hash_mode = 0;
        }
    }
    if (b.any_hash && profile_ && !b.mev[0]) {
        bool any_md5 = false;
        for (auto &p : b.pics) any_md5 |= p.codec == 1 && p.has_picture && (p.hp.hash_mode & 2) != 0;
        if (any_md5) for (auto &e : b.mev) if (hipEventCreate(&e) != hipSuccess) { (void)hipGetLastError(); e = nullptr; }
    }
    HevcBatchDims hd;
    const EnginePic *last_upload[4] = {nullptr, nullptr, nullptr, nullptr};
    b.pmask = 0;
    for (int k = 0; k < kKernelClasses; k++) { b.alg[k] = 0; b.npics[k] = 0; }
    size_t d_need = 0;
    for (auto &p : b.pics) for (auto &o : p.out) d_need += OutTables::bytes_needed(o);
    if (d_need > b.deint_cap) {
        if (b.deint_scratch) hipFree(b.deint_scratch);
        b.deint_scratch = nullptr; b.deint_cap = std::max(d_need, 2 * b.deint_cap);
        if (hipMalloc((void **)&b.deint_scratch, b.deint_cap) != hipSuccess) { (void)hipGetLastError(); b.deint_scratch = nullptr; b.deint_cap = 0; }
    }
    b.out.reset(b.deint_scratch);
    for (int i = 0; i < n; i++) {
        EnginePic &p = b.pics[i];
        const bool hevc = p.codec != 0;
        if (hevc) { b.h_hpics[i] = p.hp; if (!p.has_picture) b.h_hpics[i].stages = 0; any_hevc = true; }
        if (any_jpeg) {
            if (p.codec == 2 && p.has_picture) { b.h_jpics[i] = p.jp; max_jpeg_items = std::max(max_jpeg_items, p.jp.n_items); b.alg[7] += p.jpeg_alg_bytes; b.npics[7]++; }
            else b.h_jpics[i].n_items = 0;
        }
        b.h_pics[i] = p.pp;
        if (!p.has_picture || hevc) b.h_pics[i].stages = 0;
        else if (b.any_chain && (p.chain_ok || p.chain_intra)) {
            PicParams &q = b.h_pics[i];
            q.stages = PS_CHAIN | (p.chain_intra ? PS_CHAIN_INTRA : 0); q.chain_idx = i; q.n_deps = 0;
            if (p.chain_intra) q.want_intra_resid = 1;
            for (int k = 0; k < kMaxSurfaces; k++) q.dep_pic[k] = -1;
            bool refs_in_batch = false;
            for (int j = 0; j < i; j++) {
                const EnginePic &e = b.pics[j];
                if (e.dec != p.dec || !e.has_picture || e.codec != 0) continue;
                if (p.ref_mask & (1u << e.pp.cur)) refs_in_batch = true;
                if (e.chain_ok || e.chain_intra) { q.dep_pic[e.pp.cur] = (int8_t)j; if (p.ref_mask & (1u << e.pp.cur)) q.n_deps++; }
            }
            if (!refs_in_batch) q.stages |= PS_RECON;
        }
        stages |= b.h_pics[i].stages;
        if (p.has_picture && !hevc) max_mb_w = std::max(max_mb_w, p.mb_w);
        if (p.has_picture && ((1u << (hevc ? p.hp.cur : p.pp.cur)) & p.dec->engine_state().displayed[li])) wait_pack = true;
        if (hevc && p.has_picture) {
            const HevcPicParams &h = p.hp;
            hd.max_pus = std::max(hd.max_pus, h.n_pus); hd.max_tbs = std::max(hd.max_tbs, h.n_tbs); hd.max_itbs = std::max(hd.max_itbs, h.n_itbs);
            hd.max_ctb_w = std::max(hd.max_ctb_w, h.ctb_w); hd.max_ctb_h = std::max(hd.max_ctb_h, h.ctb_h);
            hd.max_w = std::max(hd.max_w, h.w); hd.max_h = std::max(hd.max_h, h.h); hd.any_intra |= (h.stages & HPS_INTRA) != 0;
            hd.any_deblock |= (h.stages & HPS_DEBLOCK) != 0; hd.any_sao |= (h.stages & HPS_SAO) != 0;
            if (h.hash_mode & 1) { hd.any_hash = true; b.alg[8] += (long long)h.w * h.h * 3 / 2; b.npics[8]++; }
            if (h.hash_mode & 2) { hd.any_md5 = true; b.alg[9] += (long long)h.w * h.h * 3 / 2; b.npics[9]++; }
        }
        if (p.has_picture) {
            max_mbs = std::max(max_mbs, p.mb_w * p.mb_h); max_mb_h = std::max(max_mb_h, p.mb_h);
            if (p.uploaded) { const EnginePic *&lu = last_upload[p.upload_seq % (unsigned)n_copy_]; if (!lu || p.upload_seq > lu->upload_seq) lu = &p; }
        }
        if (p.wait_prev_pack) wait_pack = true;
        for (int side : {kBefore, kAfter}) if (!b.out.add(p.out[side], side, p.disp_w, p.disp_h, p.alg_bytes[3], p.alg_bytes[4]))
            p.dec->on_engine_error("hipMalloc(deinterlace scratch) failed");
        int st = b.h_pics[i].stages;
        if (hevc && p.has_picture) { const int hs = p.hp.stages; if (hs & (HPS_MC | HPS_RESID)) { b.alg[0] += p.alg_bytes[0]; b.npics[0]++; }
            if (hs & HPS_INTRA) { b.alg[1] += p.alg_bytes[1]; b.npics[1]++; } if (hs & (HPS_DEBLOCK | HPS_SAO)) { b.alg[2] += p.alg_bytes[2]; b.npics[2]++; } }
        if (st & PS_RECON) { b.alg[0] += p.alg_bytes[0]; b.npics[0]++; }
        if (st & (PS_INTRA_LDS | PS_INTRA_V1)) { b.alg[1] += p.alg_bytes[1]; b.npics[1]++; }
        if (st & (PS_DEBLOCK_LDS | PS_DEBLOCK_V1)) { b.alg[2] += p.alg_bytes[2]; b.npics[2]++; }
        if (st & PS_CHAIN) { b.alg[4] += ((st & PS_RECON) ? 0 : p.alg_bytes[0]) + ((st & PS_CHAIN_INTRA) ? p.alg_bytes[1] : 0) + p.alg_bytes[2]; b.npics[4]++; }
    }
    b.alg[3] = b.out.alg_pack; b.npics[3] = b.out.n_frames; b.alg[5] = b.out.alg_rgb; b.npics[5] = b.out.n_rgb;
    b.alg[10] = b.out.alg_rgb444; b.npics[10] = b.out.n_chroma[0] + b.out.n_chroma[1];
    b.alg[6] = b.out.alg_deint; b.npics[6] = b.out.n_deint;
    for (auto &p : b.pics) p.dec->engine_state().displayed[li] = 0;
    for (auto &p : b.pics) p.dec->engine_state().displayed[li] |= p.out_mask;
    b.max_mbs = max_mbs; b.max_mb_h = max_mb_h; b.redo = false;
    hipStream_t st = ln.stream, pst = ln.pack_stream;
    hipStream_t ps = any_hevc ? st : ln.pre_stream;
    if (!any_hevc && (stages & (PS_INTRA_LDS | PS_DEBLOCK_LDS | PS_CHAIN))) { hipMemsetAsync(b.d_ctl, 0, sizeof(int) * (size_t)n * chain_ctl_ints(), ps);
        hipMemsetAsync(b.d_ctl + (size_t)kMaxBatch * chain_ctl_ints(), 0, chain_tail_ints() * sizeof(int), ps);
        if (stages & PS_CHAIN) {
            const double launch_ms = 0.25 * b.max_depth * std::max(1.0, max_mbs / 8160.0) + 0.8;
            const unsigned ticks = (unsigned)(std::min(100.0, std::max(10.0, 10.0 * launch_ms)) * 100000.0);
            static const unsigned forced = getenv("JM_AMD_DEC_CHAIN_WAIT_MS") ? (unsigned)(atof(getenv("JM_AMD_DEC_CHAIN_WAIT_MS")) * 100000.0) : 0u;
            hipMemsetD32Async((hipDeviceptr_t)(b.d_ctl + (size_t)kMaxBatch * chain_ctl_ints() + chain_tail_wait_limit()), (int)(forced ? forced : ticks), 1, ps);
        } }
    if (any_hevc) hipMemcpyAsync(b.d_hpics, b.h_hpics, sizeof(HevcPicParams) * n, hipMemcpyHostToDevice, ps);
    else hipMemcpyAsync(b.d_pics, b.h_pics, sizeof(PicParams) * n, hipMemcpyHostToDevice, ps);
    if (any_jpeg) hipMemcpyAsync(b.d_jpics, b.h_jpics, sizeof(JpegPicParams) * n, hipMemcpyHostToDevice, ps);
    b.out.each([&](auto &t) { for (int side : {kBefore, kAfter}) if (t.n[side])
        hipMemcpyAsync(t.dev + side * kOutSideCap, t.h(side), sizeof(*t.host) * t.n[side], hipMemcpyHostToDevice, ps); });
    for (const EnginePic *lu : last_upload) if (lu) hipStreamWaitEvent(ps, lu->uploaded, 0);
    if (profile_ && !any_hevc) hipEventRecord(b.pev[8], ps);
    bool prep_early = false;
    if (!any_hevc) {
        if (stages & (PS_DEBLOCK_LDS | PS_CHAIN)) { launch_deblock_prep(b.d_pics, n, max_mbs, ps); prep_early = true; }
        if (profile_) hipEventRecord(b.pev[9], ps);
        hipEventRecord(b.pre_done, ps);
        hipStreamWaitEvent(st, b.pre_done, 0);
    }
    if (ln.pack_hist[1]) hipStreamWaitEvent(st, ln.pack_hist[1], 0);
    if ((wait_pack || b.out.any(kBefore)) && ln.pack_hist[0]) hipStreamWaitEvent(st, ln.pack_hist[0], 0);
    auto mark = [&](int i, hipStream_t s) { if (profile_) hipEventRecord(b.pev[i], s); };
    run_side(b, kBefore, st, true);
    if (any_hevc && (hd.max_pus || hd.max_tbs || hd.any_intra || hd.any_deblock || hd.any_sao)) {
        hipEvent_t ev[5] = {b.pev[1], b.pev[2], b.pev[3], b.pev[4], b.pev[18]};
        launch_hevc_picture_batch(b.d_hpics, n, hd, b.d_progress, st, profile_ ? ev : nullptr, b.d_hash);
        if (hd.max_pus || hd.max_tbs) b.pmask |= 2;
        if (hd.any_intra) b.pmask |= 4;
        if (hd.any_deblock || hd.any_sao) b.pmask |= 8;
        b.last_ev = 4;
        if (hd.any_md5 && b.d_hash) {
            const bool timed = profile_ && b.mev[0] && b.mev[1];
            if (timed) hipEventRecord(b.mev[0], st);
            launch_hevc_md5(b.d_hpics, n, b.d_hash, st);
            if (timed) { hipEventRecord(b.mev[1], st); b.pmask |= 4096; }
        }
        if (hd.any_hash || (hd.any_md5 && b.d_hash)) hipMemcpyAsync(b.h_hash, b.d_hash, sizeof(uint32_t) * (size_t)n * kHashStride, hipMemcpyDeviceToHost, st);
        if (hd.any_hash) { b.pmask |= 2048; b.last_ev = 18; }
    }
    if (any_jpeg && max_jpeg_items > 0) {
        const bool timed = profile_ && b.jev[0] && b.jev[1];
        if (timed) hipEventRecord(b.jev[0], st);
        launch_jpeg_recon(b.d_jpics, n, max_jpeg_items, st);
        if (timed) { hipEventRecord(b.jev[1], st); b.pmask |= 1024; }
    }
    b.any_bipred = b.any_field = false;
    for (auto &p : b.pics) { b.any_bipred |= p.has_picture && p.codec == 0 && p.bipred; b.any_field |= p.has_picture && p.codec == 0 && p.pp.field != 0; }
    if (stages & PS_RECON) { launch_recon_inter(b.d_pics, n, max_mbs, b.any_bipred && !debug_no_bi_, b.any_field, b.d_err, st); b.pmask |= 2; }
    if (!any_hevc) mark(2, st);
    if (stages & PS_INTRA_LDS) { launch_intra_lds(b.d_pics, n, max_mb_h, b.d_ctl, b.d_err, st); b.pmask |= 4; }
    if (stages & PS_INTRA_V1) { launch_recon_intra(b.d_pics, n, st); b.pmask |= 4; }
    if (!any_hevc) mark(3, st);
    if ((stages & (PS_DEBLOCK_LDS | PS_CHAIN)) && !prep_early) launch_deblock_prep(b.d_pics, n, max_mbs, st);
    if (stages & PS_DEBLOCK_LDS) { launch_deblock_lds(b.d_pics, n, max_mb_h, b.d_ctl, b.d_err, debug_stall_ == 1, st); b.pmask |= 8; }
    if (stages & PS_DEBLOCK_V1) { launch_deblock(b.d_pics, n, st); b.pmask |= 8; }
    if (!any_hevc) { mark(4, st); b.last_ev = 4; }
    if (stages & PS_CHAIN) {
        const int band_rows = chain_band_rows(), L = deblock_row_lag();
        constexpr int kBandLag = 8, kKeySlack = 2, kIntraExtra = 24;
        std::vector<int> base_of(n, 0), slope_of(n, L);
        size_t n_keys = 0;
        for (int i = 0; i < n; i++) {
            if (!(b.h_pics[i].stages & PS_CHAIN)) continue;
            slope_of[i] = (b.h_pics[i].stages & PS_CHAIN_INTRA) ? 2 : L;
            for (int j = i - 1; j >= 0; j--) if (b.pics[j].dec == b.pics[i].dec && (b.h_pics[j].stages & PS_CHAIN)) {
                base_of[i] = base_of[j] + chain_lag_steps_ + kKeySlack + slope_of[i] * b.pics[i].reach_rows + b.pics[i].reach_cols +
                             kBandLag * ((b.pics[i].reach_rows + 1) / band_rows);
                if (b.h_pics[j].stages & PS_CHAIN_INTRA) base_of[i] += b.h_pics[j].mb_h + kIntraExtra;
                break; }
            n_keys = std::max(n_keys,
                (size_t)(base_of[i] + slope_of[i] * b.h_pics[i].mb_h + b.h_pics[i].mb_w + kBandLag * (b.h_pics[i].mb_h / band_rows + 1) + 2));
        }
        if (group_buckets_.size() < n_keys) group_buckets_.resize(n_keys);
        for (size_t k = 0; k < n_keys; k++) group_buckets_[k].clear();
        for (int i = 0; i < n; i++) {
            if (!(b.h_pics[i].stages & PS_CHAIN) || (b.h_pics[i].stages & PS_RECON)) continue;
            const int mb_h = b.h_pics[i].mb_h, segs = (b.h_pics[i].mb_w + 7) / 8, base = base_of[i];
            for (int r = 0; r < mb_h; r++) {
                const int kr = base + slope_of[i] * r + kBandLag * (r / band_rows);
                for (int c = 0; c < segs; c++) group_buckets_[kr + 8 * c].push_back((uint32_t)i << 16 | (uint32_t)(r * 32 + c));
            }
        }
        int n_groups = 0;
        bool with_intra = false;
        for (int i = 0; i < n; i++) if (b.h_pics[i].stages & PS_CHAIN) for (int bnd = 0; bnd * band_rows < b.h_pics[i].mb_h; bnd++) {
            if (b.h_pics[i].stages & PS_CHAIN_INTRA) { b.h_groups[n_groups++] = (uint32_t)i << 16 | 0xC000u | (uint32_t)bnd; with_intra = true; }
            b.h_groups[n_groups++] = (uint32_t)i << 16 | 0x8000u | (uint32_t)bnd;
        }
        for (size_t k = 0; k < n_keys; k++) append_bucket_by_xcd(group_buckets_[k].data(), group_buckets_[k].size(), b.h_groups, n_groups, bucket_tmp_);
        hipMemcpyAsync(b.d_groups, b.h_groups, sizeof(uint32_t) * (size_t)n_groups, hipMemcpyHostToDevice, st);
        launch_chain(b.d_pics, b.d_groups, n_groups, with_intra, b.d_ctl, b.d_err, debug_stall_ != 0, st);
        b.chain_with_intra = with_intra;
        b.pmask |= 32; mark(7, st); b.last_ev = 7;
    }
    hipEventRecord(b.kdone, st);
    hipStreamWaitEvent(pst, b.kdone, 0);
    run_side(b, kAfter, pst, true);
    hipError_t le = hipGetLastError();
    if (le != hipSuccess) fprintf(stderr, "jm_amd_dec: kernel launch failed: %s\n", hipGetErrorString(le));
    hipEventRecord(b.done, pst);
    ln.pack_hist[1] = ln.pack_hist[0]; ln.pack_hist[0] = b.packed;
}

void Engine::run_side(Batch &b, int side, hipStream_t s, bool in_launch) {
    const OutTables &t = b.out;
    auto mark = [&](int i) { if (in_launch && profile_) hipEventRecord(b.pev[i], s); };
    mark(side ? 5 : 0);
    if (t.deint.n[side]) { mark(14 + 2 * side); (t.pairs[side] ? launch_deint2 : launch_deint)(t.deint.d(side), t.deint.n[side], t.d_items, s); mark(15 + 2 * side); b.pmask |= side ? 512 : 256; }
    if (t.plain.n[side]) launch_packout(t.plain.d(side), t.plain.n[side], t.max_w, t.max_h, s);
    if (t.scale.n[side]) launch_scale_pack(t.scale.d(side), t.scale.n[side], t.s_tiles, s);
    if (t.rgb.n[side]) { mark(10 + 2 * side); launch_rgb_pack(t.rgb.d(side), t.rgb.n[side], t.r_tiles[0], t.r_tiles[1], 0, s);
        if (t.n_chroma[side]) { mark(19 + 2 * side); launch_rgb_pack(t.rgb.d(side), t.rgb.n[side], 0, 0, t.r_tiles[2], s); mark(20 + 2 * side);
            b.pmask |= side ? 16384 : 8192; }
        mark(11 + 2 * side); b.pmask |= side ? 128 : 64; }
    if (t.any(side)) b.pmask |= side ? 16 : 1;
    if (in_launch && side) { mark(6); hipEventRecord(b.packed, s); }
    if (t.any(side)) for (auto &p : b.pics) for (OutSlot *o : p.out[side].slots) if (o->dev && o->host && !o->fetch)
        hipMemcpyAsync(o->host, o->dev, o->bytes, hipMemcpyDeviceToHost, s);
    if (in_launch && !side) mark(1);
}

void Engine::recover(Lane &ln, Batch &b, const std::vector<std::pair<Decoder *, uint32_t>> &later) {
    const int n = (int)b.pics.size();
    hipStream_t st = ln.stream;
    hipStreamSynchronize(ln.pack_stream); hipStreamSynchronize(st);
    auto is_tainted = [&](Decoder *d) { return std::find(ln.tainted.begin(), ln.tainted.end(), d) != ln.tainted.end(); };
    auto taint = [&](Decoder *d) { if (!is_tainted(d)) ln.tainted.push_back(d); };
    for (int i = 0; i < n; i++) {
        Decoder *d = b.pics[i].dec;
        bool first = true;
        for (int j = 0; j < i; j++) first &= b.pics[j].dec != d;
        if (!first) continue;
        uint32_t written = 0, ext_refs = 0, shown = 0, shown_before = 0, lw = 0;
        for (int j = i; j < n; j++) {
            const EnginePic &p = b.pics[j];
            if (p.dec != d) continue;
            ext_refs |= p.ref_mask & ~written;
            shown |= p.out_mask;
            if (!p.before_empty()) shown_before |= p.out_mask;
            if (p.has_picture && p.codec == 0) written |= 1u << p.pp.cur;
        }
        for (auto &e : later) if (e.first == d) lw |= e.second;
        if ((lw & (ext_refs | shown)) || (b.redo && (written & shown_before))) taint(d);
    }
    if (b.redo && b.out.any(kBefore)) { run_side(b, kBefore, st, false); hipStreamSynchronize(st); }
    std::vector<int> depth(n, 0); int max_depth = 0;
    for (int i = 0; i < n; i++) { for (int j = 0; j < i; j++) if (b.pics[j].dec == b.pics[i].dec && b.pics[j].has_picture) depth[i]++;
        max_depth = std::max(max_depth, depth[i]); }
    for (int d = 0; d <= max_depth; d++) {
        int stages = 0;
        for (int i = 0; i < n; i++) {
            const EnginePic &p = b.pics[i];
            b.h_pics[i] = p.pp;
            b.h_pics[i].stages = (p.has_picture && p.codec == 0 && depth[i] == d) ? p.classic_stages : 0;
            stages |= b.h_pics[i].stages;
            b.h_err[i] = 0;
        }
        if (!stages) continue;
        hipMemsetAsync(b.d_ctl, 0, sizeof(int) * (size_t)n * chain_ctl_ints(), st);
        hipMemcpyAsync(b.d_pics, b.h_pics, sizeof(PicParams) * n, hipMemcpyHostToDevice, st);
        if (stages & PS_RECON) launch_recon_inter(b.d_pics, n, b.max_mbs, b.any_bipred, b.any_field, b.d_err, st);
        if (stages & PS_INTRA_LDS) launch_intra_lds(b.d_pics, n, b.max_mb_h, b.d_ctl, b.d_err, st);
        if (stages & PS_INTRA_V1) launch_recon_intra(b.d_pics, n, st);
        if (stages & PS_DEBLOCK_LDS) { launch_deblock_prep(b.d_pics, n, b.max_mbs, st);
            launch_deblock_lds(b.d_pics, n, b.max_mb_h, b.d_ctl, b.d_err, false, st); }
        if (stages & PS_DEBLOCK_V1) launch_deblock(b.d_pics, n, st);
        hipStreamSynchronize(st);
    }
    if (b.out.any(kAfter)) { run_side(b, kAfter, st, false); hipStreamSynchronize(st); }
    for (int i = 0; i < n; i++) if (is_tainted(b.pics[i].dec) && !b.h_err[i]) b.h_err[i] = kErrNotRecovered;
    { std::lock_guard<std::mutex> lk(sm_); st_.chain_recoveries++; }
    const auto since_epoch = std::chrono::steady_clock::now().time_since_epoch();
    chain_block_until_ns_ = std::chrono::duration_cast<std::chrono::nanoseconds>(since_epoch).count() + 30ll * 1000 * 1000 * 1000;
    static bool said = false;
    if (!said) { said = true;
        fprintf(stderr, "jm_amd_dec: device %d: a chain launch ran out of time waiting for workgroups (is the GPU shared?) -- its pictures were decoded "
                "again by the stage kernels; chain launches pause for 30 s\n", device_);
    }
}

void Engine::dump_chain_state(Batch &b) {
    const int n = (int)b.pics.size(), stride = chain_ctl_ints();
    std::vector<int> ctl((size_t)kMaxBatch * stride + chain_tail_ints());
    if (hipMemcpy(ctl.data(), b.d_ctl, ctl.size() * sizeof(int), hipMemcpyDeviceToHost) != hipSuccess) { (void)hipGetLastError(); return; }
    const int *lw = ctl.data() + (size_t)kMaxBatch * stride;
    int n_band_wgs = 0, n_recon_groups = 0;
    for (int i = 0; i < n; i++) if (b.h_pics[i].stages & PS_CHAIN) { const int bands = (b.h_pics[i].mb_h + 15) / 16;
        n_band_wgs += ((b.h_pics[i].stages & PS_CHAIN_INTRA) ? 4 : 2) * bands;
        if (!(b.h_pics[i].stages & PS_RECON)) n_recon_groups += b.h_pics[i].mb_h * ((b.h_pics[i].mb_w + 7) / 8); }
    fprintf(stderr, "  census: abort %d | reconstruction workgroups started %d done %d (work list: %d groups x 2, some empty) | "
        "band workgroups started %d done %d of %d | highest work-list index started %d | band budget %d / %d\n",
        lw[0], lw[1], lw[2], n_recon_groups, lw[3], lw[4], n_band_wgs, lw[5], chain_bands_max_, chain_bands_max_intra_);
    if (lw[2] > 0) fprintf(stderr, "  reconstruction workgroups: %.2f us each on average, of which %.2f us in wait_final (wave 0)\n",
        0.01 * (double)(unsigned)lw[7] / lw[2], 0.01 * (double)(unsigned)lw[6] / lw[2]);
    if (lw[8]) fprintf(stderr,
        "  FIRST give-up (of %d): code %d (1 fin: reconstruction waits for the deblocking of picture `pic`; 2 bits: a deblocking band of `pic` waits "
        "for its reconstruction; 4 ring; 8 intra ring; 16 ifin) pic %d where 0x%x (fin: band << 16 | macroblock column; bits: row << 16 | column, bit 31 of "
        "the row = intra band; ring: band << 16 | chroma) needed %d saw %d / %d\n", lw[8], lw[9], lw[10], (unsigned)lw[11], lw[12], lw[13], lw[14]);
    if (lw[8]) fprintf(stderr,
        "  ... the same counter read by an atomic read-modify-write when the wait gave up: %d (equal to what the polls saw = the producer stood there; larger = "
        "published and not seen) | waiter: XCC %d, HW_ID1 0x%08x (wave %d SIMD %d CU %d SA %d SE %d), %d looks | its timer skipped %d clock gap(s), the longest "
        "%.2f ms | wait limit of the launch %.1f ms\n", lw[16], lw[17] & 15, (unsigned)lw[18], lw[18] & 31, (lw[18] >> 8) & 3, (lw[18] >> 10) & 15,
        (lw[18] >> 16) & 1, (lw[18] >> 18) & 7, lw[19], lw[20], lw[21] * 1e-5, lw[15] * 1e-5);
    for (int i = 0; i < n; i++) {
        const PicParams &q = b.h_pics[i];
        if (!(q.stages & PS_CHAIN)) continue;
        const int *c = ctl.data() + (size_t)i * stride;
        const int bands = (q.mb_h + 15) / 16;
        fprintf(stderr, "  picture %2d dec %p %dx%d stages 0x%x%s deps %d err %d reach %d/%d |", i, (void *)b.pics[i].dec, q.mb_w, q.mb_h, q.stages,
            (q.stages & PS_RECON) ? " (reconstructed before the launch)" : "", q.n_deps, b.h_err[i], b.pics[i].reach_rows, b.pics[i].reach_cols);
        for (int k = 0; k < bands; k++) fprintf(stderr, " b%d ring %d/%d fin %d/%d", k, c[0 + k], c[32 + k], c[64 + k], c[64 + 32 + k]);
        if (q.stages & PS_CHAIN_INTRA) for (int k = 0; k < bands; k++) fprintf(stderr, " i%d ring %d/%d ifin %d/%d", k, c[128 + k], c[128 + 32 + k], c[192 + k],
            c[192 + 32 + k]);
        int full = 0, first_open = -1, first_open_bits = 0;
        for (int r = 0; r < q.mb_h; r++) { int cnt = 0; for (int w = 0; w < 8; w++) cnt += __builtin_popcount((unsigned)c[256 + r * 8 + w]);
            if (cnt >= q.mb_w) full++; else if (first_open < 0) { first_open = r; first_open_bits = cnt; } }
        fprintf(stderr, " | bitmap: %d of %d rows complete, first open row %d has %d of %d\n", full, q.mb_h, first_open, first_open_bits, q.mb_w);
    }
    const int *ts = lw + chain_tail_head_ints();
    int t0 = 0x7fffffff;
    for (int i = 0; i < n; i++) for (int k = 0; k < 4; k += 2) if (ts[4 * i + k]) t0 = std::min(t0, 0x40000000 - ts[4 * i + k]);
    if (t0 != 0x7fffffff) for (int i = 0; i < n; i++) {
        if (!(b.h_pics[i].stages & PS_CHAIN)) continue;
        auto us = [&](int k) { const int v = ts[4 * i + k]; return v ? ((k & 1) ? v - t0 : 0x40000000 - v - t0) * 0.01 : -1.0; };
        fprintf(stderr, "  time line picture %2d dec %p: reconstruction %.1f .. %.1f us, bands %.1f .. %.1f us\n", i, (void *)b.pics[i].dec, us(0), us(1),
            us(2), us(3));
    }
}

void Engine::complete(Lane &ln, Batch &b, bool failed) {
    LANE_TRACE("retire lane %d batch %llu pics %zu\n", (int)(&ln - lanes_), b.serial, b.pics.size());
    if (!failed && (b.redo || b.any_chain)) {
        bool wait_err = b.redo;
        for (size_t i = 0; i < b.pics.size(); i++) wait_err |= b.h_err[i] != 0 && b.any_chain;
        if (wait_err) {
            static std::atomic<int> dumped{0};
            if (getenv("JM_AMD_DEC_VERBOSE") || (!b.redo && dumped.fetch_add(1) < 4)) {
                fprintf(stderr, "jm_amd_dec: chain launch of %zu pictures gave up%s; codes:", b.pics.size(), b.redo ? " (redo of the batch behind one that did)" : "");
                for (size_t i = 0; i < b.pics.size(); i++) fprintf(stderr, " %d", b.h_err[i]); fprintf(stderr, "\n");
                dump_chain_state(b); }
            std::vector<std::pair<Decoder *, uint32_t>> later;
            if (!b.redo) ln.tainted.clear();
            if (ln.inflight > 1) {
                Batch &nx = ln.ring[(ln.tail + 1) % kBatchRing]; hipEventSynchronize(nx.done); nx.redo = true;
                for (auto &p : nx.pics) if (p.has_picture && p.codec == 0) later.emplace_back(p.dec, 1u << p.pp.cur);
            }
            recover(ln, b, later);
        }
    }
    if (profile_ && !failed) {
        std::lock_guard<std::mutex> lk(sm_);
        auto add = [&](int cls, int e0, int e1, bool ran) {
            if (!ran) return;
            float ms = 0;
            if (hipEventElapsedTime(&ms, b.pev[e0], b.pev[e1]) == hipSuccess) { st_.ns[cls] += ms * 1e6; st_.launches[cls]++; }
        };
        add(3, 0, 1, b.pmask & 1); add(0, 1, 2, b.pmask & 2); add(1, 2, 3, b.pmask & 4); add(2, 3, 4, b.pmask & 8); add(3, 5, 6, b.pmask & 16);
        add(4, 4, 7, b.pmask & 32); add(5, 10, 11, b.pmask & 64); add(5, 12, 13, b.pmask & 128);
        add(6, 14, 15, b.pmask & 256); add(6, 16, 17, b.pmask & 512); add(8, 4, 18, b.pmask & 2048);
        add(10, 19, 20, b.pmask & 8192); add(10, 21, 22, b.pmask & 16384);
        if (b.pmask & 1024) { float ms = 0; if (hipEventElapsedTime(&ms, b.jev[0], b.jev[1]) == hipSuccess) { st_.ns[7] += ms * 1e6; st_.launches[7]++; } }
        if (b.pmask & 4096) { float ms = 0; if (hipEventElapsedTime(&ms, b.mev[0], b.mev[1]) == hipSuccess) { st_.ns[9] += ms * 1e6; st_.launches[9]++; } }
        for (int k = 0; k < kKernelClasses; k++) { st_.pics[k] += b.npics[k]; st_.alg_bytes[k] += b.alg[k]; }
        st_.batches++; st_.batch_pics += (long long)b.pics.size();
        const int li = (int)(&ln - lanes_);
        st_.lane_batches[li]++; st_.lane_pics[li] += (long long)b.pics.size();
        if (b.last_ev >= 0) {
            float ms = 0;
            if (hipEventElapsedTime(&ms, b.pev[0], b.pev[b.last_ev]) == hipSuccess) st_.lane_busy_ns[li] += ms * 1e6;
            const Batch &pb = ln.ring[(ln.tail + kBatchRing - 1) % kBatchRing];
            if (pb.serial + 1 == b.serial && pb.last_ev >= 0 && hipEventElapsedTime(&ms, pb.pev[pb.last_ev], b.pev[0]) == hipSuccess && ms > 0) {
                st_.lane_gap_ns[li] += ms * 1e6;
                float mu = 0, mp = 0;
                const bool h264 = !b.pics.empty() && b.pics[0].codec == 0;
                if (h264 && !b.launched_dry && hipEventElapsedTime(&mu, pb.pev[pb.last_ev], b.pev[8]) == hipSuccess && mu > 0) st_.lane_upwait_ns[li] += std::min(mu, ms) * 1e6;
                if (h264 && !b.launched_dry && hipEventElapsedTime(&mp, pb.pev[pb.last_ev], b.pev[9]) == hipSuccess && mp > 0) st_.lane_prewait_ns[li] += std::min(mp, ms) * 1e6;
            }
        }
        (void)hipGetLastError();
    }
    if (b.any_chain && !failed) { static const bool timeline = getenv("JM_AMD_DEC_CHAIN_TIMELINE") != nullptr;
        if (timeline) { fprintf(stderr, "jm_amd_dec: chain launch of %zu pictures\n", b.pics.size()); dump_chain_state(b); } }
    if (b.h_err[kMaxBatch]) { std::lock_guard<std::mutex> lk(sm_); st_.wait_gap_launches++; st_.wait_gap_max_ticks = std::max(st_.wait_gap_max_ticks,
        (long long)(unsigned)b.h_err[kMaxBatch + 1]);
        if (getenv("JM_AMD_DEC_VERBOSE")) fprintf(stderr, "jm_amd_dec: a chain launch's waits saw %d clock gap(s), the longest %.2f ms: its waves were not run meanwhile "
            "(chain launch %lld of this process, batch %llu of its lane, %.1f ms after the engine's first trace point, CLOCK_MONOTONIC %.3f s when it retired)\n",
            b.h_err[kMaxBatch], (unsigned)b.h_err[kMaxBatch + 1] * 1e-5, st_.chain_batches + 1, b.serial, trace_ms(),
            std::chrono::duration<double>(std::chrono::steady_clock::now().time_since_epoch()).count());
        b.h_err[kMaxBatch] = b.h_err[kMaxBatch + 1] = 0; }
    if (b.any_chain && !failed) { static const bool census = getenv("JM_AMD_DEC_CENSUS") != nullptr;
        if (census) { int tail[32];
            if (hipMemcpy(tail, b.d_ctl + (size_t)kMaxBatch * chain_ctl_ints(), sizeof tail, hipMemcpyDeviceToHost) == hipSuccess) {
                std::lock_guard<std::mutex> lk(sm_); st_.quad_windows += tail[22]; st_.private_windows += tail[23]; }
            else (void)hipGetLastError(); } }
    if (b.any_chain && !failed) { std::lock_guard<std::mutex> lk(sm_); st_.chain_batches++; st_.chain_i_batches += b.chain_with_intra;
        for (auto &p : b.pics) st_.chain_pics += p.has_picture && (p.chain_ok || p.chain_intra); }
    { std::lock_guard<std::mutex> lk(m_); const int li = (int)(&ln - lanes_);
      for (auto &p : b.pics) { p.dec->engine_state().inflight--; p.dec->engine_state().lane_inflight[li]--; } pending_gen_++; }
    for (size_t i = 0; i < b.pics.size(); i++) if (b.h_err[i]) { b.pics[i].dec->on_device_wait_error(b.h_err[i]); b.h_err[i] = 0;
        std::lock_guard<std::mutex> lk(sm_); st_.wait_errors++; }
    for (size_t i = 0; i < b.pics.size(); i++) {
        const EnginePic &p = b.pics[i];
        if (p.codec != 1 || (p.hash_type <= 0 && !p.hash_md5)) continue;
        if (failed || b.redo || !p.has_picture || !p.hp.hash_mode || !b.h_hash) { p.dec->on_picture_hash(p, nullptr, -1); continue; }
        if (p.hash_md5) {
            const uint8_t *digests = (const uint8_t *)(b.h_hash + i * kHashStride + kMd5Word);
            int bad = -1;
            for (int c = 2; c >= 0; c--) if (memcmp(digests + 16 * c, p.md5_want[c], 16) != 0) bad = c;
            p.dec->on_picture_md5(p, digests, bad);
            continue;
        }
        const uint32_t *words = b.h_hash + i * kHashStride, *got = words + (p.hash_type == 1 ? 0 : 3);
        int bad = -1;
        for (int c = 2; c >= 0; c--) if (got[c] != p.hash_want[c]) bad = c;
        p.dec->on_picture_hash(p, words, bad);
    }
    for (auto &p : b.pics) p.dec->on_engine_done(p, failed);
    b.pics.clear();
}

void Engine::look_for_other_users() {
    if (!kfd_gpu_id_) return;
    const long long now = std::chrono::duration_cast<std::chrono::nanoseconds>(std::chrono::steady_clock::now().time_since_epoch()).count();
    const bool was = gpu_shared_.load(std::memory_order_relaxed);
    if (now - shared_checked_ns_.load() <= (was ? 200ll : 1000ll) * 1000 * 1000) return;
    shared_checked_ns_ = now;
    const bool sh = kfd_gpu_has_other_users(kfd_gpu_id_);
    if (sh != was) fprintf(stderr, "jm_amd_dec: device %d: %s -- chain launches %s\n", device_,
        sh ? "another process has compute queues on this GPU" : "the GPU is no longer shared", sh ? "off" : "on again");
    gpu_shared_.store(sh, std::memory_order_relaxed);
}

void Engine::run() {
    hipSetDevice(device_);
    { const char *e = getenv("JM_AMD_DEC_TIMER_SLACK_NS"); const unsigned long ns = e ? strtoul(e, nullptr, 10) : 0ul; if (ns) prctl(PR_SET_TIMERSLACK, ns, 0, 0, 0); }
    for (;;) {
        bool progressed = false;
        for (auto &ln : lanes_) {
            while (ln.inflight > 0) {
                const hipError_t q = hipEventQuery(ln.ring[ln.tail].done);
                if (q == hipErrorNotReady) break;
                if (q != hipSuccess && !device_failed_) { device_failed_ = true;
                    fprintf(stderr, "jm_amd_dec: device %d failed: %s -- every handle on it now returns errors\n", device_, hipGetErrorString(q)); }
                { auto t0 = std::chrono::steady_clock::now(); complete(ln, ln.ring[ln.tail], q != hipSuccess);
                    long long ns = std::chrono::duration_cast<std::chrono::nanoseconds>(std::chrono::steady_clock::now() - t0).count();
                    std::lock_guard<std::mutex> lk(sm_); st_.complete_ns += ns; }
                ln.tail = (ln.tail + 1) % kBatchRing; ln.inflight--;
                progressed = true;
            }
        }
        lingered_ = false;
        for (int li = 0; li < kLanes; li++) {
            Lane &ln = lanes_[li];
            static const int max_inflight = getenv("JM_AMD_DEC_INFLIGHT") ? atoi(getenv("JM_AMD_DEC_INFLIGHT")) : 2;
            if (ln.inflight >= (li == kIntraLane && early_intra_ && deep_queues_ ? 1 : max_inflight)) continue;
            Batch &b = ln.ring[ln.head];
            bool have;
            if (li == kOrdinaryLane) { bool any; { std::lock_guard<std::mutex> lk(m_); any = !pending_.empty(); } if (any) look_for_other_users(); }
            { std::lock_guard<std::mutex> lk(m_); have = !pending_.empty() && form(ln, li, b); }
            if (!have) continue;
            if (device_failed_) { complete(ln, b, true); progressed = true; continue; }
            { auto t0 = std::chrono::steady_clock::now(); launch(ln, b);
                long long ns = std::chrono::duration_cast<std::chrono::nanoseconds>(std::chrono::steady_clock::now() - t0).count();
                std::lock_guard<std::mutex> lk(sm_); st_.launch_ns += ns; }
            ln.head = (ln.head + 1) % kBatchRing; ln.inflight++;
            progressed = true;
        }
        if (progressed) continue;
        bool busy = false;
        for (auto &ln : lanes_) busy |= ln.inflight > 0;
        if (busy || lingered_) std::this_thread::sleep_for(std::chrono::microseconds(20));
        else { std::unique_lock<std::mutex> lk(m_); cv_.wait_for(lk, std::chrono::milliseconds(2), [&] { return !pending_.empty(); }); }
    }
}

}
```

### jmcodec_amd/csrc/engine.h

```cpp
#pragma once
#include "jobs.h"
#include "out_tables.h"
#include "hevc_jobs.h"
#include "jpeg_jobs.h"
#include <atomic>
#include <condition_variable>
#include <deque>
#include <mutex>
#include <string>
#include <thread>
#include <vector>

struct ihipStream_t; struct ihipEvent_t;

namespace jmamd {

class Decoder;

constexpr int kBatchRing = 4;
constexpr int kMaxChainGroups = 128 * 1024;
constexpr int kMaxChainBands = 384;
constexpr int kMaxChainBandsIntra = 256;
constexpr int kMinChainLag = 24;
constexpr int kOrdinaryLane = 0;
constexpr int kIntraLane = 1;
constexpr int kErrNotRecovered = 32;
constexpr int kLanes = 4;
constexpr int kHevcLane = 2;
constexpr int kHevcIntraLane = 3;
constexpr int kEarlyIntraAhead = 10;

struct EnginePic {
    Decoder *dec = nullptr;
    bool has_picture = false;
    PicParams pp;
    int codec = 0;
    HevcPicParams hp;
    JpegPicParams jp; long long jpeg_alg_bytes = 0;
    int job_slot = -1;
    ihipEvent_t *uploaded = nullptr; unsigned long long upload_seq = 0;
    OutSide out[2];
    bool before_empty() const { return out[kBefore].frames() == 0; }
    int mb_w = 0, mb_h = 0, disp_w = 0, disp_h = 0;
    bool wait_prev_pack = false;
    bool chain_ok = false;
    bool chain_intra = false;
    int classic_stages = 0;
    uint32_t ref_mask = 0, out_mask = 0;
    bool bipred = false;
    int reach_rows = 0;
    int reach_cols = 0;
    long long alg_bytes[5] = {0, 0, 0, 0, 0};
    unsigned long long seq = 0;
    int hash_type = 0, hash_poc = 0; uint32_t hash_want[3] = {0, 0, 0};
    bool hash_md5 = false; uint8_t md5_want[3][16] = {};
    int lane(bool chaining = false) const {
        if (codec == 2) return kHevcLane;
        if (codec == 1) return (has_picture && hp.n_pus == 0 && hp.n_itbs > 0) ? kHevcIntraLane : kHevcLane;
        return (has_picture && (pp.stages & PS_INTRA_LDS) && !(chaining && chain_intra)) ? kIntraLane : kOrdinaryLane;
    }
};

constexpr int kKernelClasses = 11;
struct EngineStats {
    double ns[kKernelClasses] = {}; long long launches[kKernelClasses] = {}, pics[kKernelClasses] = {}, alg_bytes[kKernelClasses] = {};
    long long batches = 0, batch_pics = 0, chain_batches = 0, chain_pics = 0, wait_errors = 0, chain_recoveries = 0;
    long long chain_i_batches = 0;
    long long forms = 0, form_decoders = 0, form_pending = 0;
    long long launch_ns = 0, complete_ns = 0;
    long long rej_other_lane = 0, rej_cross_lane = 0, rej_tables = 0;
    long long wait_gap_launches = 0, wait_gap_max_ticks = 0;
    long long quad_windows = 0, private_windows = 0;
    long long early_intra = 0;
    long long blocked_ns = 0, blocked_n = 0;
    double lane_upwait_ns[4] = {0, 0, 0, 0}, lane_prewait_ns[4] = {0, 0, 0, 0}; long long lane_dry[4] = {0, 0, 0, 0};
    double lane_busy_ns[4] = {0, 0, 0, 0}, lane_gap_ns[4] = {0, 0, 0, 0}; long long lane_batches[4] = {0, 0, 0, 0}, lane_pics[4] = {0, 0, 0, 0};
};

struct EngineDecoderState {
    int inflight = 0;
    int lane_inflight[4] = {0, 0, 0, 0};
    uint32_t displayed[4] = {0, 0, 0, 0};
    unsigned long long next_seq = 0;
    int n_pending = 0;
    unsigned long long form_tag = 0;
    unsigned long long scan_tag = 0; uint32_t scan_touched = 0; int scan_ahead = 0; bool scan_closed = false;
    long long blocked_since = 0;
    int in_batch = 0; uint32_t batch_written = 0, batch_read = 0; bool batch_stop = false;
};

void mem_trace(const char *tag);

class Engine {
public:
    static Engine *get(int device);
    void submit(EnginePic &&p);
    unsigned long long upload(uint8_t *dev, const uint8_t *host, size_t n, ihipEvent_t *ev, bool spread = true);
    void set_profile(bool on) { profile_ = on; }
    int  fetchers() const { return fetchers_.load(std::memory_order_relaxed); }
    void fetch_begin() { fetchers_.fetch_add(1, std::memory_order_relaxed); }
    void fetch_end() { fetchers_.fetch_sub(1, std::memory_order_relaxed); }
    bool set_knob(const std::string &key, long long v);
    EngineStats stats();
    int device() const { return device_; }
    bool gpu_shared() const { return gpu_shared_.load(std::memory_order_relaxed); }

private:
    explicit Engine(int device);
    void run();
    struct Batch {
        PicParams *h_pics = nullptr, *d_pics = nullptr;
        HevcPicParams *h_hpics = nullptr, *d_hpics = nullptr;
        JpegPicParams *h_jpics = nullptr, *d_jpics = nullptr; ihipEvent_t *jev[2] = {nullptr, nullptr};
        int *d_progress = nullptr;
        int *d_ctl = nullptr;
        int *h_err = nullptr, *d_err = nullptr;
        uint32_t *d_hash = nullptr, *h_hash = nullptr; bool any_hash = false;
        ihipEvent_t *mev[2] = {nullptr, nullptr};
        bool any_chain = false, chain_with_intra = false, redo = false; int max_depth = 1;
        int max_mbs = 0, max_mb_h = 0; bool any_bipred = false, any_field = false;
        uint32_t *h_groups = nullptr, *d_groups = nullptr;
        OutTables out;
        uint8_t *deint_scratch = nullptr; size_t deint_cap = 0;
        ihipEvent_t *done = nullptr, *kdone = nullptr, *packed = nullptr, *pre_done = nullptr, *pev[23] = {nullptr};
        std::vector<EnginePic> pics;
        unsigned pmask = 0;
        long long alg[kKernelClasses] = {}; int npics[kKernelClasses] = {};
        int last_ev = -1;
        bool launched_dry = false;
        unsigned long long serial = 0;
    };
    struct Lane {
        ihipStream_t *stream = nullptr, *pack_stream = nullptr, *pre_stream = nullptr;
        ihipEvent_t *pack_hist[2] = {nullptr, nullptr};
        Batch ring[kBatchRing];
        int head = 0, tail = 0, inflight = 0;
        unsigned long long launched = 0;
        long long wait_since_ns = 0;
        std::vector<Decoder *> tainted;
    };
    bool form(Lane &ln, int lane_idx, Batch &b);
    bool cross_lane_ = true, early_intra_ = true;
    long long fill_linger_ns_ = 4000 * 1000;
    unsigned long long scan_tag_form_ = 0;
    bool lingered_ = false;
    int decoders_pending_ = 0;
    bool deep_queues_ = false;
    std::atomic<int> early_intra_ahead_{kEarlyIntraAhead};
    long long early_scan_ns_ = 0; unsigned long long early_scan_tag_ = 0;
    unsigned long long pending_gen_ = 0, early_scanned_gen_ = ~0ull;
    bool others_done(Decoder *d, int lane_idx, unsigned long long seq);
    void inflight_masks(Decoder *d, uint32_t &touched);
    std::atomic<int> chain_max_streams_{16};
    int chain_bands_max_ = kMaxChainBands, chain_bands_max_intra_ = kMaxChainBandsIntra;
    std::atomic<int> chain_depth_{8}, chain_lag_steps_{24};
    std::atomic<int> chain_depth_few_{16};
    struct Recent { Decoder *dec; long long t; int mbs; };
    std::vector<Recent> recent_;
    std::vector<std::vector<uint32_t>> group_buckets_;
    std::vector<uint32_t> bucket_tmp_;
    void launch(Lane &ln, Batch &b);
    void run_side(Batch &b, int side, ihipStream_t *s, bool in_launch);
    void complete(Lane &ln, Batch &b, bool failed);
    void dump_chain_state(Batch &b);
    void recover(Lane &ln, Batch &b, const std::vector<std::pair<Decoder *, uint32_t>> &later);

    int device_, numa_node_ = -1;
    unsigned kfd_gpu_id_ = 0; std::atomic<bool> gpu_shared_{false}; std::atomic<long long> shared_checked_ns_{0};
    void look_for_other_users();
    ihipStream_t *copy_streams_[4] = {nullptr, nullptr, nullptr, nullptr}; int n_copy_ = 2;
    std::mutex um_; unsigned long long upload_seq_ = 0;
    Lane lanes_[kLanes];
    std::mutex m_; std::condition_variable cv_;
    std::deque<EnginePic> pending_;
    bool profile_ = false, ok_ = false, device_failed_ = false;
    std::atomic<int> debug_stall_{0};
    std::atomic<int> debug_no_bi_{0};
    std::atomic<int> fetchers_{0};
    std::atomic<long long> chain_block_until_ns_{0};
    int chain_linger_streams_ = 2;
    std::mutex sm_; EngineStats st_;
    std::thread th_;
};

}
```

### jmcodec_amd/csrc/jobs.h

```cpp
#pragma once
#include <stddef.h>
#include <stdint.h>
#include <vector>

namespace jmamd {

enum : uint8_t { MB_INTER = 0, MB_I4 = 1, MB_I16 = 2, MB_PCM = 3 };

enum : uint8_t {
    MBF_AVAIL_A = 1,
    MBF_AVAIL_B = 2,
    MBF_AVAIL_C = 4,
    MBF_AVAIL_D = 8,
    MBF_CB_DC   = 16,
    MBF_CR_DC   = 32,
    MBF_MV_EXT  = 64,
    MBF_DECODED = 128,
};

enum : uint8_t { MBM_T8X8 = 16, MBM_BIPRED = 32 };
constexpr int kBiRecInt16 = 72;

struct MbRec {
    uint8_t  kind;
    uint8_t  qp;
    uint8_t  modes;
    uint8_t  flags;
    uint16_t cbp_blk;
    uint8_t  cbp_cac;
    uint8_t  slice;
    uint32_t coef_off;
    int8_t   ref[4];
    union {
        int16_t  mv[4][2];
        uint8_t  i4[8];
        uint32_t mv_ext;
    } u;
};
static_assert(sizeof(MbRec) == 32, "MbRec must stay 32 bytes");


constexpr int kMaxSlicesPerPicture = 255;

struct SliceRec {
    int8_t  alpha_off;
    int8_t  beta_off;
    uint8_t disable;
    uint8_t pad;
};

struct SliceWp {
    uint8_t mode;
    uint8_t logwd_y, logwd_c, pad;
    int16_t w[2][16][3];
    int8_t  o[2][16][3];
    uint8_t imp_w1[16][16];
};
static_assert(sizeof(SliceWp) == 4 + 192 + 96 + 256, "SliceWp layout");

constexpr int kMaxSurfaces = 20;

struct PicParams {
    int mb_w, mb_h;
    uint32_t mb_w_magic;
    uint32_t surf_stride;
    int field;
    int pitch;
    int chroma_offset;
    int cb_qp_off, cr_qp_off;
    int n_slices;
    int cur;
    uint8_t *surf[kMaxSurfaces];
    uint8_t *surf_base;
    const MbRec *mbs;
    const SliceRec *slices;
    const int16_t *mv_ext;
    const int16_t *coef;
    int16_t *resid;
    void *dbrec;
    int want_intra_resid;
    int stages;
    const SliceWp *wp;
    int flat_scaling;
    uint8_t wscale4[6][16];
    uint8_t wscale8[2][64];
    int chain_idx;
    int n_deps;
    int8_t dep_pic[kMaxSurfaces];
};

enum : int { PS_RECON = 1, PS_INTRA_LDS = 2, PS_INTRA_V1 = 4, PS_DEBLOCK_LDS = 8, PS_DEBLOCK_V1 = 16,
             PS_CHAIN = 32,
             PS_CHAIN_INTRA = 64 };

struct PackJob {
    const uint8_t *src; uint8_t *dst;
    int pitch, chroma_offset, width, height, out_fmt;
    int lone_field;
};

struct ScaleAxis {
    const int32_t *first; const int16_t *w;
    int taps, src_len;
};
constexpr int kScaleMaxTaps = 9;
struct ScaleJob {
    const uint8_t *src; uint8_t *dst;
    int pitch, chroma_offset;
    int crop_x, crop_y;
    int tw, th, out_fmt;
    int lone_field;
    ScaleAxis ax[4];
    int rx, ry, rw, rh;
    int fill;
};

enum : int { RGB_U8 = 0, RGB_F32 = 1, RGB_F16 = 2, RGB_BF16 = 3 };
struct RgbJob {
    ScaleJob s;
    int identity;
    int cy, crv, cgu, cgv, cbu;
    int yo;
    int dtype, planar, bgr;
    float k[3], b[3];
    int fill;
    int chroma;
    ScaleAxis cax[2];
};

struct DeintJob {
    const uint8_t *src; uint8_t *dst;
    int pitch, chroma_offset, width, height;
    int dst_pitch, dst_chroma_offset;
    int out_fmt;
    int mode;
    int parity;
    int thr;
    uint8_t *dst2;
};
struct DeintReq { DeintJob job; int feeds, index, index2;
    bool pair() const { return feeds ? index2 != 0 : job.dst2 != nullptr; } };

struct OutSlot;
struct OutSide {
    std::vector<PackJob> plain;
    std::vector<ScaleJob> scale;
    std::vector<RgbJob> rgb;
    std::vector<DeintReq> deint;
    std::vector<OutSlot *> slots;
    size_t frames() const { size_t n = plain.size() + scale.size() + rgb.size(); for (auto &r : deint) if (r.feeds == 0) n += r.pair() ? 2 : 1; return n; }
};

}
```

### jmcodec_amd/csrc/kernels.h

```cpp
#pragma once
#include <hip/hip_runtime_api.h>
#include "jobs.h"

namespace jmamd {
void launch_recon_inter(const PicParams *d_pics, int n, int max_mbs, bool any_bipred, bool any_field, int *d_err, hipStream_t st);
void launch_recon_intra(const PicParams *d_pics, int n, hipStream_t st);
void launch_deblock(const PicParams *d_pics, int n, hipStream_t st);
constexpr int kMaxMbRows = 1056;
bool intra_lds_supported(int mb_w, int mb_h);
void launch_intra_lds(const PicParams *d_pics, int n, int max_mb_h, int *ctl, int *err, hipStream_t st);
bool deblock_lds_supported(int mb_w, int mb_h);
constexpr int kDeblockMaxBands = 32, kDeblockProgressStride = 2 * kDeblockMaxBands;
void launch_deblock_prep(const PicParams *d_pics, int n, int max_mbs, hipStream_t st);
void launch_deblock_lds(const PicParams *d_pics, int n, int max_mb_h, int *ctl, int *err, bool debug_stall, hipStream_t st);
bool chain_supported(int mb_w, int mb_h);
void launch_chain(const PicParams *d_pics, const uint32_t *d_groups, int n_groups, bool with_intra, int *ctl, int *err, bool debug_stall, hipStream_t st);
int  chain_band_rows();
int  deblock_row_lag();
int  chain_resident_workgroups(bool intra);
int  chain_ctl_ints();
int  chain_tail_head_ints(); int chain_tail_wait_limit();
int  chain_tail_ints();
void launch_packout(const PackJob *d_jobs, int n, int max_width, int max_height, hipStream_t st);
int  scale_tiles(int tw, int th);
void launch_scale_pack(const ScaleJob *d_jobs, int n, int max_tiles, hipStream_t st);
int  rgb_tiles(int tw, int th);
void launch_rgb_pack(const RgbJob *d_jobs, int n, int identity_tiles, int scaled_tiles, int chroma_tiles, hipStream_t st);
int  deint_items(int w, int h);
void launch_deint(const DeintJob *d_jobs, int n, int max_items, hipStream_t st);
int  deint2_items(int w, int h);
void launch_deint2(const DeintJob *d_jobs, int n, int max_items, hipStream_t st);
void launch_frame_to_argb(const uint8_t *d_src, int w, int h, int fmt, uint8_t *d_dst, int dst_pitch, hipStream_t st);
void launch_frame_to_nv12_pitch(const uint8_t *d_src, int w, int h, int fmt, uint8_t *d_dst, int pitch, hipStream_t st);
}
```

Before: 15240.

## Fuse intra prediction and deblocking into one persistent kernel on the intra lane

Adds a k_intra_deblock kernel where half of the workgroups run intra band reconstruction and the other half run deblocking of the same bands. The two roles synchronise through the chain control rings, replacing separate intra and deblock launches for intra-lane batches. The engine admits pictures into a fused batch only while the workgroup count fits resident occupancy. It adds a timeout fallback that re-decodes with the stage kernels and pauses fusing when the GPU is shared. It is on by default and adds a spin-wait deadlock risk plus extra scheduling logic.

```diff
diff --git a/jmcodec_amd/csrc/deblock_lds.hip b/jmcodec_amd/csrc/deblock_lds.hip
--- a/jmcodec_amd/csrc/deblock_lds.hip
+++ b/jmcodec_amd/csrc/deblock_lds.hip
@@ -10,7 +10,7 @@
 
 __global__ __launch_bounds__(256) void k_deblock_prep(const PicParams *pics) {
     const PicParams &pp = pics[blockIdx.y];
-    if (!(pp.stages & (PS_DEBLOCK_LDS | PS_CHAIN))) return;
+    if (!(pp.stages & (PS_DEBLOCK_LDS | PS_CHAIN | PS_FUSED_DEBLOCK))) return;
     DbRec *out = (DbRec *)pp.dbrec;
     const int per_xcd = ((int)gridDim.x + 7) >> 3;
     const int blk = ((int)blockIdx.x & 7) * per_xcd + ((int)blockIdx.x >> 3);
diff --git a/jmcodec_amd/csrc/decoder.cpp b/jmcodec_amd/csrc/decoder.cpp
--- a/jmcodec_amd/csrc/decoder.cpp
+++ b/jmcodec_amd/csrc/decoder.cpp
@@ -161,7 +161,7 @@
         chroma_loc_opt_ = (int)v;
     }
     else if (k == "profile") { profile_ = v != 0; if (engine_) engine_->set_profile(profile_); }
-    else if (k.rfind("chain_", 0) == 0 || k == "debug_stall" || k == "debug_no_bi" || k == "early_intra_ahead") {
+    else if (k.rfind("chain_", 0) == 0 || k == "debug_stall" || k == "debug_no_bi" || k == "early_intra_ahead" || k == "intra_fused") {
         if (!engine_ || !engine_->set_knob(k, v)) return -1;
     }
     else if (k == "wait_idle") {
@@ -309,6 +309,8 @@
         if (k == "eng_rej_cross_lane") return es.rej_cross_lane;
         if (k == "eng_rej_tables") return es.rej_tables;
         if (k == "eng_early_intra") return es.early_intra;
+        if (k == "eng_intra_fused_batches") return es.intra_fused_batches;
+        if (k == "eng_intra_fused_pics") return es.intra_fused_pics;
         if (k == "eng_blocked_ns") return es.blocked_ns;
         if (k == "eng_blocked_n") return es.blocked_n;
         for (int i = 0; i < 4; i++) {
@@ -1686,6 +1688,7 @@
         ep.chain_intra = chain_ok_ && chain_intra_on_ && t->n_intra > 0 && use_lds_intra_ && (t->n_i8x8 == 0 || lds_intra8_) && (pp.stages & PS_DEBLOCK_LDS) &&
                          !t->field;
         ep.classic_stages = pp.stages;
+        ep.fuse_ok = chain_ok_ && chain_intra_on_ && (pp.stages & PS_INTRA_LDS) && !(pp.stages & PS_DEBLOCK_V1) && !t->field;
         for (auto &sl : t->slices) ep.bipred |= sl.refs.bipred_rec;
         ep.reach_rows = ((t->max_mvy >> 2) + 15) / 16;
         ep.reach_cols = ((t->max_mvx >> 2) + 15) / 16;
diff --git a/jmcodec_amd/csrc/engine.cpp b/jmcodec_amd/csrc/engine.cpp
--- a/jmcodec_amd/csrc/engine.cpp
+++ b/jmcodec_amd/csrc/engine.cpp
@@ -52,6 +52,7 @@
     if (const char *e = getenv("JM_AMD_DEC_CROSS_LANE")) cross_lane_ = atoi(e) != 0;
     if (const char *e = getenv("JM_AMD_DEC_FILL_LINGER_US")) fill_linger_ns_ = std::max(0, atoi(e)) * 1000ll;
     if (const char *e = getenv("JM_AMD_DEC_EARLY_INTRA")) early_intra_ = atoi(e) != 0;
+    if (const char *e = getenv("JM_AMD_DEC_INTRA_FUSED")) intra_fused_ = atoi(e) != 0;
     if (hipSetDevice(device_) != hipSuccess) return;
     if (const char *e = getenv("JM_AMD_DEC_COPY_STREAMS")) n_copy_ = std::max(1, std::min(atoi(e), 4));
     int prio_lo = 0, prio_hi = 0, copy_prio = 0;
@@ -99,6 +100,10 @@
       if (getenv("JM_AMD_DEC_VERBOSE")) fprintf(stderr,
           "jm_amd_dec: device %d holds %d / %d chain workgroups (plain / with the intra role): band budget %d / %d\n", device_, r, ri, chain_bands_max_,
           chain_bands_max_intra_); }
+    { const int r = intra_deblock_resident_workgroups();
+      fused_wgs_max_ = r / 2;
+      if (getenv("JM_AMD_DEC_VERBOSE")) fprintf(stderr, "jm_amd_dec: device %d holds %d workgroups of k_intra_deblock: a fused launch takes up to %d\n", device_, r,
+          fused_wgs_max_); }
     mem_trace("engine: occupancy queries");
     ok_ = true;
     numa_node_ = numa_node_of_device(device_, true);
@@ -137,16 +142,24 @@
 }
 
 bool Engine::set_knob(const std::string &key, long long v) {
-    if (key.rfind("chain_", 0) == 0) { chain_block_until_ns_ = 0; shared_checked_ns_ = 0; }
+    if (key.rfind("chain_", 0) == 0 || key == "intra_fused") { chain_block_until_ns_ = 0; shared_checked_ns_ = 0; }
     if (key == "chain_depth") { if (v <= 0) { chain_depth_ = 8; chain_depth_few_ = 16; }
         else { chain_depth_ = (int)std::min(v, 16ll); chain_depth_few_ = chain_depth_.load(); } }
     else if (key == "chain_lag") chain_lag_steps_ = (int)std::max((long long)kMinChainLag, std::min(v, 1024ll));
     else if (key == "chain_streams") chain_max_streams_ = (int)std::max(0ll, v);
     else if (key == "debug_stall") debug_stall_ = (int)v;
+    else if (key == "intra_fused") intra_fused_ = v != 0;
     else if (key == "debug_no_bi") debug_no_bi_ = (int)v;
     else if (key == "early_intra_ahead") early_intra_ahead_ = (int)std::max(1ll, std::min(v, 64ll));
     else return false;
     return true;
+}
+
+bool Engine::fusing_now(bool chaining) const {
+    if (chaining || !intra_fused_.load(std::memory_order_relaxed) || fused_wgs_max_ <= 0 || debug_stall_.load(std::memory_order_relaxed) != 0) return false;
+    if (gpu_shared_.load(std::memory_order_relaxed)) return false;
+    const long long now = std::chrono::duration_cast<std::chrono::nanoseconds>(std::chrono::steady_clock::now().time_since_epoch()).count();
+    return now >= chain_block_until_ns_.load(std::memory_order_relaxed);
 }
 
 EngineStats Engine::stats() { std::lock_guard<std::mutex> lk(sm_); return st_; }
@@ -160,6 +173,7 @@
             bool mine = false;
             for (auto &p : ob.pics) if (p.dec == d && p.seq < seq) { mine = true; break; }
             if (mine && hipEventQuery(ob.packed) != hipSuccess) { (void)hipGetLastError(); return false; }
+            if (mine && ob.n_fused > 0) for (size_t i = 0; i < ob.pics.size(); i++) if (ob.h_err[i]) return false;
         }
     }
     return true;
@@ -174,7 +188,7 @@
 }
 
 bool Engine::form(Lane &ln, int lane_idx, Batch &b) {
-    b.pics.clear(); b.any_chain = false; b.chain_with_intra = false; b.max_depth = 1;
+    b.pics.clear(); b.any_chain = false; b.chain_with_intra = false; b.max_depth = 1; b.n_fused = 0;
     bool chaining = false;
     int depth_now = chain_depth_;
     {
@@ -239,6 +253,14 @@
         n_pre += p.out[kBefore].frames(); n_post += p.out[kAfter].frames();
     };
     const size_t n_dec_pending = (size_t)decoders_pending_;
+    const bool fusing = lane_idx == kIntraLane && fusing_now(chaining);
+    int fused_n = 0, fused_bands = 0;
+    b.fuse = fusing;
+    auto fused_fits = [&](const EnginePic &p) {
+        if (!fusing || p.codec != 0 || !p.has_picture || !p.fuse_ok || fused_n == 0) return true;
+        return 4 * std::max(fused_bands, (p.mb_h + 15) / 16) * (fused_n + 1) <= fused_wgs_max_; };
+    auto fused_took = [&](const EnginePic &p) { if (fusing && p.codec == 0 && p.has_picture && p.fuse_ok) { fused_n++;
+        fused_bands = std::max(fused_bands, (p.mb_h + 15) / 16); } };
     auto took = [&](EngineDecoderState &es) { if (--es.n_pending == 0) decoders_pending_--; };
     for (auto it = pending_.begin(); it != pending_.end() && (int)b.pics.size() < kMaxBatch && seen.size() < n_dec_pending;) {
         Decoder *d = it->dec;
@@ -249,6 +271,7 @@
         if (it->lane(chaining) != lane_idx) why = 1;
         else if (es.inflight > es.lane_inflight[lane_idx] && !(relaxed && others_done(d, lane_idx, it->seq))) why = 2;
         else if (n_pre + it->out[kBefore].frames() > (size_t)kOutSideCap || n_post + it->out[kAfter].frames() > (size_t)kOutSideCap) why = 3;
+        else if (!fused_fits(*it)) why = 4;
         if (why) {
             if (lane_idx == kOrdinaryLane && it->codec == 0) { std::lock_guard<std::mutex> lk(sm_);
                 (why == 1 ? st_.rej_other_lane : why == 2 ? st_.rej_cross_lane : st_.rej_tables)++;
@@ -269,6 +292,7 @@
         es.inflight++; es.lane_inflight[lane_idx]++;
         es.in_batch = 1; es.batch_written = es.batch_read = 0; es.batch_stop = false;
         account(*it, es);
+        fused_took(*it);
         members.push_back(d);
         took(es);
         b.pics.push_back(std::move(*it));
@@ -300,7 +324,8 @@
             for (auto &c : cand) pos.push_back((size_t)(c - pending_.begin()));
             for (size_t k = pos.size(); k-- > 0 && (int)b.pics.size() < kMaxBatch;) {
                 auto it = pending_.begin() + (std::ptrdiff_t)pos[k];
-                if (n_post + it->out[kAfter].frames() > (size_t)kOutSideCap) continue;
+                if (n_post + it->out[kAfter].frames() > (size_t)kOutSideCap || !fused_fits(*it)) continue;
+                fused_took(*it);
                 EngineDecoderState &es = it->dec->engine_state();
                 es.inflight++; es.lane_inflight[lane_idx]++;
                 LANE_TRACE("early dec %p seq %llu\n", (void *)it->dec, it->seq);
@@ -385,7 +410,8 @@
             if (ended) { std::lock_guard<std::mutex> lk(sm_); st_.lane_dry[li]++; } }
     }
     LANE_TRACE("launch lane %d batch %llu pics %d\n", li, b.serial, n);
-    int max_mbs = 0, max_mb_h = 0, max_mb_w = 0, stages = 0;
+    int max_mbs = 0, max_mb_h = 0, max_mb_w = 0, stages = 0, fused_bands = 0, fused_mb_h = 0;
+    b.n_fused = 0;
     bool wait_pack = false, any_hevc = false, any_jpeg = false; int max_jpeg_items = 0;
     for (auto &p : b.pics) any_jpeg |= p.codec == 2 && p.has_picture;
     if (any_jpeg && !b.h_jpics) {
@@ -450,6 +476,12 @@
             }
             if (!refs_in_batch) q.stages |= PS_RECON;
         }
+        else if (b.fuse && p.fuse_ok && (p.classic_stages & PS_INTRA_LDS) && 4 * std::max(fused_bands, (p.mb_h + 15) / 16) * (b.n_fused + 1) <= fused_wgs_max_) {
+            PicParams &q = b.h_pics[i];
+            q.stages = PS_RECON | PS_FUSED | ((p.classic_stages & PS_DEBLOCK_LDS) ? PS_FUSED_DEBLOCK : 0); q.chain_idx = i; q.n_deps = 0;
+            for (int k = 0; k < kMaxSurfaces; k++) q.dep_pic[k] = -1;
+            b.n_fused++; fused_bands = std::max(fused_bands, (p.mb_h + 15) / 16); fused_mb_h = std::max(fused_mb_h, p.mb_h);
+        }
         stages |= b.h_pics[i].stages;
         if (p.has_picture && !hevc) max_mb_w = std::max(max_mb_w, p.mb_w);
         if (p.has_picture && ((1u << (hevc ? p.hp.cur : p.pp.cur)) & p.dec->engine_state().displayed[li])) wait_pack = true;
@@ -475,6 +507,7 @@
         if (st & PS_RECON) { b.alg[0] += p.alg_bytes[0]; b.npics[0]++; }
         if (st & (PS_INTRA_LDS | PS_INTRA_V1)) { b.alg[1] += p.alg_bytes[1]; b.npics[1]++; }
         if (st & (PS_DEBLOCK_LDS | PS_DEBLOCK_V1)) { b.alg[2] += p.alg_bytes[2]; b.npics[2]++; }
+        if (st & PS_FUSED) { b.alg[1] += p.alg_bytes[1] + ((st & PS_FUSED_DEBLOCK) ? p.alg_bytes[2] : 0); b.npics[1]++; }
         if (st & PS_CHAIN) { b.alg[4] += ((st & PS_RECON) ? 0 : p.alg_bytes[0]) + ((st & PS_CHAIN_INTRA) ? p.alg_bytes[1] : 0) + p.alg_bytes[2]; b.npics[4]++; }
     }
     b.alg[3] = b.out.alg_pack; b.npics[3] = b.out.n_frames; b.alg[5] = b.out.alg_rgb; b.npics[5] = b.out.n_rgb;
@@ -485,13 +518,16 @@
     b.max_mbs = max_mbs; b.max_mb_h = max_mb_h; b.redo = false;
     hipStream_t st = ln.stream, pst = ln.pack_stream;
     hipStream_t ps = any_hevc ? st : ln.pre_stream;
-    if (!any_hevc && (stages & (PS_INTRA_LDS | PS_DEBLOCK_LDS | PS_CHAIN))) { hipMemsetAsync(b.d_ctl, 0, sizeof(int) * (size_t)n * chain_ctl_ints(), ps);
+    if (!any_hevc && (stages & (PS_INTRA_LDS | PS_DEBLOCK_LDS | PS_CHAIN | PS_FUSED))) { hipMemsetAsync(b.d_ctl, 0, sizeof(int) * (size_t)n * chain_ctl_ints(), ps);
         hipMemsetAsync(b.d_ctl + (size_t)kMaxBatch * chain_ctl_ints(), 0, chain_tail_ints() * sizeof(int), ps);
         if (stages & PS_CHAIN) {
             const double launch_ms = 0.25 * b.max_depth * std::max(1.0, max_mbs / 8160.0) + 0.8;
             const unsigned ticks = (unsigned)(std::min(100.0, std::max(10.0, 10.0 * launch_ms)) * 100000.0);
             static const unsigned forced = getenv("JM_AMD_DEC_CHAIN_WAIT_MS") ? (unsigned)(atof(getenv("JM_AMD_DEC_CHAIN_WAIT_MS")) * 100000.0) : 0u;
             hipMemsetD32Async((hipDeviceptr_t)(b.d_ctl + (size_t)kMaxBatch * chain_ctl_ints() + chain_tail_wait_limit()), (int)(forced ? forced : ticks), 1, ps);
+        } else if (stages & PS_FUSED) {
+            const unsigned ticks = (unsigned)(std::min(100.0, std::max(10.0, 11.0 * std::max(1.0, max_mbs / 8160.0))) * 100000.0);
+            hipMemsetD32Async((hipDeviceptr_t)(b.d_ctl + (size_t)kMaxBatch * chain_ctl_ints() + chain_tail_wait_limit()), (int)ticks, 1, ps);
         } }
     if (any_hevc) hipMemcpyAsync(b.d_hpics, b.h_hpics, sizeof(HevcPicParams) * n, hipMemcpyHostToDevice, ps);
     else hipMemcpyAsync(b.d_pics, b.h_pics, sizeof(PicParams) * n, hipMemcpyHostToDevice, ps);
@@ -502,7 +538,7 @@
     if (profile_ && !any_hevc) hipEventRecord(b.pev[8], ps);
     bool prep_early = false;
     if (!any_hevc) {
-        if (stages & (PS_DEBLOCK_LDS | PS_CHAIN)) { launch_deblock_prep(b.d_pics, n, max_mbs, ps); prep_early = true; }
+        if (stages & (PS_DEBLOCK_LDS | PS_CHAIN | PS_FUSED_DEBLOCK)) { launch_deblock_prep(b.d_pics, n, max_mbs, ps); prep_early = true; }
         if (profile_) hipEventRecord(b.pev[9], ps);
         hipEventRecord(b.pre_done, ps);
         hipStreamWaitEvent(st, b.pre_done, 0);
@@ -540,10 +576,11 @@
     if (stages & PS_INTRA_LDS) { launch_intra_lds(b.d_pics, n, max_mb_h, b.d_ctl, b.d_err, st); b.pmask |= 4; }
     if (stages & PS_INTRA_V1) { launch_recon_intra(b.d_pics, n, st); b.pmask |= 4; }
     if (!any_hevc) mark(3, st);
-    if ((stages & (PS_DEBLOCK_LDS | PS_CHAIN)) && !prep_early) launch_deblock_prep(b.d_pics, n, max_mbs, st);
+    if ((stages & (PS_DEBLOCK_LDS | PS_CHAIN | PS_FUSED_DEBLOCK)) && !prep_early) launch_deblock_prep(b.d_pics, n, max_mbs, st);
     if (stages & PS_DEBLOCK_LDS) { launch_deblock_lds(b.d_pics, n, max_mb_h, b.d_ctl, b.d_err, debug_stall_ == 1, st); b.pmask |= 8; }
     if (stages & PS_DEBLOCK_V1) { launch_deblock(b.d_pics, n, st); b.pmask |= 8; }
     if (!any_hevc) { mark(4, st); b.last_ev = 4; }
+    if (stages & PS_FUSED) { mark(23, st); launch_intra_deblock(b.d_pics, n, fused_mb_h, b.d_ctl, b.d_err, st); mark(24, st); b.pmask |= 32768; b.last_ev = 24; }
     if (stages & PS_CHAIN) {
         const int band_rows = chain_band_rows(), L = deblock_row_lag();
         constexpr int kBandLag = 8, kKeySlack = 2, kIntraExtra = 24;
@@ -663,8 +700,8 @@
     chain_block_until_ns_ = std::chrono::duration_cast<std::chrono::nanoseconds>(since_epoch).count() + 30ll * 1000 * 1000 * 1000;
     static bool said = false;
     if (!said) { said = true;
-        fprintf(stderr, "jm_amd_dec: device %d: a chain launch ran out of time waiting for workgroups (is the GPU shared?) -- its pictures were decoded "
-                "again by the stage kernels; chain launches pause for 30 s\n", device_);
+        fprintf(stderr, "jm_amd_dec: device %d: a chain launch (or a fused launch of the intra lane) ran out of time waiting for workgroups (is the GPU "
+                "shared?) -- its pictures were decoded again by the stage kernels; such launches pause for 30 s\n", device_);
     }
 }
 
@@ -693,13 +730,13 @@
         (lw[18] >> 16) & 1, (lw[18] >> 18) & 7, lw[19], lw[20], lw[21] * 1e-5, lw[15] * 1e-5);
     for (int i = 0; i < n; i++) {
         const PicParams &q = b.h_pics[i];
-        if (!(q.stages & PS_CHAIN)) continue;
+        if (!(q.stages & (PS_CHAIN | PS_FUSED))) continue;
         const int *c = ctl.data() + (size_t)i * stride;
         const int bands = (q.mb_h + 15) / 16;
         fprintf(stderr, "  picture %2d dec %p %dx%d stages 0x%x%s deps %d err %d reach %d/%d |", i, (void *)b.pics[i].dec, q.mb_w, q.mb_h, q.stages,
             (q.stages & PS_RECON) ? " (reconstructed before the launch)" : "", q.n_deps, b.h_err[i], b.pics[i].reach_rows, b.pics[i].reach_cols);
         for (int k = 0; k < bands; k++) fprintf(stderr, " b%d ring %d/%d fin %d/%d", k, c[0 + k], c[32 + k], c[64 + k], c[64 + 32 + k]);
-        if (q.stages & PS_CHAIN_INTRA) for (int k = 0; k < bands; k++) fprintf(stderr, " i%d ring %d/%d ifin %d/%d", k, c[128 + k], c[128 + 32 + k], c[192 + k],
+        if (q.stages & (PS_CHAIN_INTRA | PS_FUSED)) for (int k = 0; k < bands; k++) fprintf(stderr, " i%d ring %d/%d ifin %d/%d", k, c[128 + k], c[128 + 32 + k], c[192 + k],
             c[192 + 32 + k]);
         int full = 0, first_open = -1, first_open_bits = 0;
         for (int r = 0; r < q.mb_h; r++) { int cnt = 0; for (int w = 0; w < 8; w++) cnt += __builtin_popcount((unsigned)c[256 + r * 8 + w]);
@@ -719,13 +756,13 @@
 
 void Engine::complete(Lane &ln, Batch &b, bool failed) {
     LANE_TRACE("retire lane %d batch %llu pics %zu\n", (int)(&ln - lanes_), b.serial, b.pics.size());
-    if (!failed && (b.redo || b.any_chain)) {
+    if (!failed && (b.redo || b.any_chain || b.n_fused > 0)) {
         bool wait_err = b.redo;
-        for (size_t i = 0; i < b.pics.size(); i++) wait_err |= b.h_err[i] != 0 && b.any_chain;
+        for (size_t i = 0; i < b.pics.size(); i++) wait_err |= b.h_err[i] != 0 && (b.any_chain || b.n_fused > 0);
         if (wait_err) {
             static std::atomic<int> dumped{0};
             if (getenv("JM_AMD_DEC_VERBOSE") || (!b.redo && dumped.fetch_add(1) < 4)) {
-                fprintf(stderr, "jm_amd_dec: chain launch of %zu pictures gave up%s; codes:", b.pics.size(), b.redo ? " (redo of the batch behind one that did)" : "");
+                fprintf(stderr, "jm_amd_dec: %s launch of %zu pictures gave up%s; codes:", b.n_fused > 0 ? "fused intra" : "chain", b.pics.size(), b.redo ? " (redo of the batch behind one that did)" : "");
                 for (size_t i = 0; i < b.pics.size(); i++) fprintf(stderr, " %d", b.h_err[i]); fprintf(stderr, "\n");
                 dump_chain_state(b); }
             std::vector<std::pair<Decoder *, uint32_t>> later;
@@ -747,7 +784,7 @@
         add(3, 0, 1, b.pmask & 1); add(0, 1, 2, b.pmask & 2); add(1, 2, 3, b.pmask & 4); add(2, 3, 4, b.pmask & 8); add(3, 5, 6, b.pmask & 16);
         add(4, 4, 7, b.pmask & 32); add(5, 10, 11, b.pmask & 64); add(5, 12, 13, b.pmask & 128);
         add(6, 14, 15, b.pmask & 256); add(6, 16, 17, b.pmask & 512); add(8, 4, 18, b.pmask & 2048);
-        add(10, 19, 20, b.pmask & 8192); add(10, 21, 22, b.pmask & 16384);
+        add(10, 19, 20, b.pmask & 8192); add(10, 21, 22, b.pmask & 16384); add(1, 23, 24, b.pmask & 32768);
         if (b.pmask & 1024) { float ms = 0; if (hipEventElapsedTime(&ms, b.jev[0], b.jev[1]) == hipSuccess) { st_.ns[7] += ms * 1e6; st_.launches[7]++; } }
         if (b.pmask & 4096) { float ms = 0; if (hipEventElapsedTime(&ms, b.mev[0], b.mev[1]) == hipSuccess) { st_.ns[9] += ms * 1e6; st_.launches[9]++; } }
         for (int k = 0; k < kKernelClasses; k++) { st_.pics[k] += b.npics[k]; st_.alg_bytes[k] += b.alg[k]; }
@@ -782,6 +819,7 @@
             if (hipMemcpy(tail, b.d_ctl + (size_t)kMaxBatch * chain_ctl_ints(), sizeof tail, hipMemcpyDeviceToHost) == hipSuccess) {
                 std::lock_guard<std::mutex> lk(sm_); st_.quad_windows += tail[22]; st_.private_windows += tail[23]; }
             else (void)hipGetLastError(); } }
+    if (b.n_fused > 0 && !failed) { std::lock_guard<std::mutex> lk(sm_); st_.intra_fused_batches++; st_.intra_fused_pics += b.n_fused; }
     if (b.any_chain && !failed) { std::lock_guard<std::mutex> lk(sm_); st_.chain_batches++; st_.chain_i_batches += b.chain_with_intra;
         for (auto &p : b.pics) st_.chain_pics += p.has_picture && (p.chain_ok || p.chain_intra); }
     { std::lock_guard<std::mutex> lk(m_); const int li = (int)(&ln - lanes_);
@@ -845,7 +883,7 @@
             if (ln.inflight >= (li == kIntraLane && early_intra_ && deep_queues_ ? 1 : max_inflight)) continue;
             Batch &b = ln.ring[ln.head];
             bool have;
-            if (li == kOrdinaryLane) { bool any; { std::lock_guard<std::mutex> lk(m_); any = !pending_.empty(); } if (any) look_for_other_users(); }
+            if (li == kOrdinaryLane || li == kIntraLane) { bool any; { std::lock_guard<std::mutex> lk(m_); any = !pending_.empty(); } if (any) look_for_other_users(); }
             { std::lock_guard<std::mutex> lk(m_); have = !pending_.empty() && form(ln, li, b); }
             if (!have) continue;
             if (device_failed_) { complete(ln, b, true); progressed = true; continue; }
diff --git a/jmcodec_amd/csrc/engine.h b/jmcodec_amd/csrc/engine.h
--- a/jmcodec_amd/csrc/engine.h
+++ b/jmcodec_amd/csrc/engine.h
@@ -46,6 +46,7 @@
     bool chain_ok = false;
     bool chain_intra = false;
     int classic_stages = 0;
+    bool fuse_ok = false;
     uint32_t ref_mask = 0, out_mask = 0;
     bool bipred = false;
     int reach_rows = 0;
@@ -71,6 +72,7 @@
     long long rej_other_lane = 0, rej_cross_lane = 0, rej_tables = 0;
     long long wait_gap_launches = 0, wait_gap_max_ticks = 0;
     long long quad_windows = 0, private_windows = 0;
+    long long intra_fused_batches = 0, intra_fused_pics = 0;
     long long early_intra = 0;
     long long blocked_ns = 0, blocked_n = 0;
     double lane_upwait_ns[4] = {0, 0, 0, 0}, lane_prewait_ns[4] = {0, 0, 0, 0}; long long lane_dry[4] = {0, 0, 0, 0};
@@ -118,11 +120,13 @@
         uint32_t *d_hash = nullptr, *h_hash = nullptr; bool any_hash = false;
         ihipEvent_t *mev[2] = {nullptr, nullptr};
         bool any_chain = false, chain_with_intra = false, redo = false; int max_depth = 1;
+        bool fuse = false;
+        int n_fused = 0;
         int max_mbs = 0, max_mb_h = 0; bool any_bipred = false, any_field = false;
         uint32_t *h_groups = nullptr, *d_groups = nullptr;
         OutTables out;
         uint8_t *deint_scratch = nullptr; size_t deint_cap = 0;
-        ihipEvent_t *done = nullptr, *kdone = nullptr, *packed = nullptr, *pre_done = nullptr, *pev[23] = {nullptr};
+        ihipEvent_t *done = nullptr, *kdone = nullptr, *packed = nullptr, *pre_done = nullptr, *pev[25] = {nullptr};
         std::vector<EnginePic> pics;
         unsigned pmask = 0;
         long long alg[kKernelClasses] = {}; int npics[kKernelClasses] = {};
@@ -151,6 +155,9 @@
     unsigned long long pending_gen_ = 0, early_scanned_gen_ = ~0ull;
     bool others_done(Decoder *d, int lane_idx, unsigned long long seq);
     void inflight_masks(Decoder *d, uint32_t &touched);
+    std::atomic<int> intra_fused_{1};
+    int fused_wgs_max_ = 0;
+    bool fusing_now(bool chaining) const;
     std::atomic<int> chain_max_streams_{16};
     int chain_bands_max_ = kMaxChainBands, chain_bands_max_intra_ = kMaxChainBandsIntra;
     std::atomic<int> chain_depth_{8}, chain_lag_steps_{24};
diff --git a/jmcodec_amd/csrc/intra_deblock.hip b/jmcodec_amd/csrc/intra_deblock.hip
--- /dev/null
+++ b/jmcodec_amd/csrc/intra_deblock.hip
@@ -0,0 +1,47 @@
+#include <hip/hip_runtime.h>
+#include "jobs.h"
+#include "kernels.h"
+#include "kernel_common.h"
+#include "chain_common.h"
+#include "deblock_device.h"
+#include "intra_device.h"
+
+namespace jmamd {
+
+int deblock_depth();
+int deblock_pub();
+
+constexpr int kIntraDeblockSmemBytes = kIntraSmemBytes > kDeblockSmemBytes ? kIntraSmemBytes : kDeblockSmemBytes;
+static_assert(kIBandRows == kBandRows, "both roles cut a plane into the same bands");
+
+template <int DEPTH>
+__global__ __launch_bounds__(256) __attribute__((flatten)) void k_intra_deblock(const PicParams *pics, int *ctl, int *err, int pub) {
+    __shared__ __align__(16) uint8_t smem[kIntraDeblockSmemBytes];
+    const PicParams &pp = pics[blockIdx.y];
+    if (!(pp.stages & PS_FUSED)) return;
+    const int per_role = (int)gridDim.x >> 1;
+    const bool deblock = (int)blockIdx.x >= per_role;
+    const int idx = (int)blockIdx.x - (deblock ? per_role : 0), band = idx >> 1;
+    const bool is_chroma = (idx & 1) != 0;
+    int *cpic = ctl + (size_t)pp.chain_idx * kChainStride;
+    if (!deblock) intra_band_body<true>(pp, band, is_chroma, cpic + kChainIntraRing, smem, cpic, err + pp.chain_idx);
+    else if (pp.stages & PS_FUSED_DEBLOCK) deblock_band_body<DEPTH, true, true>(pp, band, is_chroma, cpic + kChainRing, pub, smem, cpic, err + pp.chain_idx);
+}
+
+int intra_deblock_resident_workgroups() {
+    int per_cu = 0, dev = 0; hipDeviceProp_t prop;
+    if (hipGetDevice(&dev) != hipSuccess || hipGetDeviceProperties(&prop, dev) != hipSuccess) return 0;
+    const bool d2 = deblock_depth() <= 2;
+    if ((d2 ? hipOccupancyMaxActiveBlocksPerMultiprocessor(&per_cu, k_intra_deblock<2>, 256, 0)
+            : hipOccupancyMaxActiveBlocksPerMultiprocessor(&per_cu, k_intra_deblock<3>, 256, 0)) != hipSuccess) { (void)hipGetLastError(); return 0; }
+    return per_cu * prop.multiProcessorCount;
+}
+
+void launch_intra_deblock(const PicParams *d_pics, int n, int max_mb_h, int *ctl, int *err, hipStream_t st) {
+    const int bands = (max_mb_h + kBandRows - 1) / kBandRows, pub = deblock_pub();
+    dim3 grid(4 * bands, n), block(256);
+    if (deblock_depth() <= 2) hipLaunchKernelGGL((k_intra_deblock<2>), grid, block, 0, st, d_pics, ctl, err, pub);
+    else hipLaunchKernelGGL((k_intra_deblock<3>), grid, block, 0, st, d_pics, ctl, err, pub);
+}
+
+}
diff --git a/jmcodec_amd/csrc/jobs.h b/jmcodec_amd/csrc/jobs.h
--- a/jmcodec_amd/csrc/jobs.h
+++ b/jmcodec_amd/csrc/jobs.h
@@ -91,7 +91,8 @@
 
 enum : int { PS_RECON = 1, PS_INTRA_LDS = 2, PS_INTRA_V1 = 4, PS_DEBLOCK_LDS = 8, PS_DEBLOCK_V1 = 16,
              PS_CHAIN = 32,
-             PS_CHAIN_INTRA = 64 };
+             PS_CHAIN_INTRA = 64,
+             PS_FUSED = 128, PS_FUSED_DEBLOCK = 256 };
 
 struct PackJob {
     const uint8_t *src; uint8_t *dst;
diff --git a/jmcodec_amd/csrc/kernels.h b/jmcodec_amd/csrc/kernels.h
--- a/jmcodec_amd/csrc/kernels.h
+++ b/jmcodec_amd/csrc/kernels.h
@@ -18,6 +18,8 @@
 int  chain_band_rows();
 int  deblock_row_lag();
 int  chain_resident_workgroups(bool intra);
+void launch_intra_deblock(const PicParams *d_pics, int n, int max_mb_h, int *ctl, int *err, hipStream_t st);
+int  intra_deblock_resident_workgroups();
 int  chain_ctl_ints();
 int  chain_tail_head_ints(); int chain_tail_wait_limit();
 int  chain_tail_ints();
```

After: 15210. No clear change (-0.2%).
